# google/bayesnf

Measured on AMD Instinct MI355X. Metric: train-steps/sec x ensemble_size (member-steps/s, whole job), higher is better.
Workload: dtype bf16; 1 GPU; C2 chickenpox-like MAP: N=10232 rows, D=3, F=57, width=512, depth=2, NORMAL, full batch, lr=0.005; members_per_gpu=64, ensemble_size=64, parallelism=ensemble-shard x1 (no data-path collective)

## Files before the change

bayesnf_amd/_native.py:

```python

from __future__ import annotations

import ctypes as C
import os

import numpy as np

from . import spec as _spec

_LIB_NAME = 'libbnf_hip.so'
_lib = None

ABI_VERSION = 6
MAX_INPUTS, MAX_GROUPS, MAX_LAYERS, MAX_FREQS, MAX_INTERACT = 8, 12, 8, 96, 16
DTYPE = {'fp32': 0, 'f32': 0, 'float32': 0, 'fp32_exact': 0, 'fp32_split': 3, 'bf16x3': 3, 'bf16': 1, 'bfloat16': 1, 'fp8': 2}
DTYPE_NAME = {0: 'fp32', 1: 'bf16', 2: 'fp8', 3: 'fp32_split'}
OBS = {'NORMAL': 0, 'NB': 1, 'ZINB': 2}
MODE_MAP, MODE_VI = 0, 1
PIPELINE = {'auto': 0, 'layers': 1, 'panel': 3}

EXPORTS = (
    'bnf_abi_version', 'bnf_last_error', 'bnf_create', 'bnf_destroy',
    'bnf_workspace_bytes', 'bnf_state_bytes', 'bnf_param_bytes', 'bnf_owned_bytes', 'bnf_bind',
    'bnf_init_params', 'bnf_init_params_keys', 'bnf_train', 'bnf_row_tables', 'bnf_row_keys', 'bnf_vi_posterior_draws', 'bnf_vi_noise_keys', 'bnf_forward',
    'bnf_normal_mixture_quantiles', 'bnf_count_mixture_quantiles', 'bnf_debug_loss_and_grad',
    'bnf_debug_row_index', 'bnf_debug_vi_eps', 'bnf_debug_vi_noise', 'bnf_debug_activation',
    'bnf_debug_gemm_nt', 'bnf_debug_gemm_tn', 'bnf_debug_poison_lds', 'bnf_profile_enable', 'bnf_profile_read',
    'bnf_kernel_flops', 'bnf_comm_available', 'bnf_comm_unique_id', 'bnf_comm_create', 'bnf_allgather',
    'bnf_comm_create_local', 'bnf_allgather_group', 'bnf_comm_destroy')


class BnfConfig(C.Structure):
  _fields_ = [
      ('abi_version', C.c_int32), ('device', C.c_int32), ('dtype', C.c_int32),
      ('obs_model', C.c_int32), ('mode', C.c_int32),
      ('n_inputs', C.c_int32), ('width', C.c_int32), ('depth', C.c_int32),
      ('n_features', C.c_int32), ('n_params', C.c_int32),
      ('n_groups', C.c_int32),
      ('group_kind', C.c_int32 * MAX_GROUPS),
      ('group_arg', C.c_int32 * MAX_GROUPS),
      ('group_ncols', C.c_int32 * MAX_GROUPS),
      ('group_col0', C.c_int32 * MAX_GROUPS),
      ('group_scale_off', C.c_int32 * MAX_GROUPS),
      ('fourier_degree', C.c_int32 * MAX_INPUTS),
      ('input_scale', C.c_float * MAX_INPUTS),
      ('n_freqs', C.c_int32),
      ('freq', C.c_float * MAX_FREQS),
      ('harmonic', C.c_float * MAX_FREQS),
      ('n_interact', C.c_int32),
      ('interact', (C.c_int32 * 2) * MAX_INTERACT),
      ('off_log_noise_scale', C.c_int32), ('off_shape', C.c_int32),
      ('off_inflated', C.c_int32),
      ('off_bias', C.c_int32 * (MAX_LAYERS + 1)),
      ('off_kernel', C.c_int32 * (MAX_LAYERS + 1)),
      ('off_layer_scale', C.c_int32 * MAX_LAYERS),
      ('off_output_scale', C.c_int32), ('off_lsa', C.c_int32),
      ('off_act_weight', C.c_int32),
      ('n_rows', C.c_int64), ('batch', C.c_int64),
      ('members', C.c_int32), ('member_offset', C.c_int64),
      ('vi_samples', C.c_int32), ('forward_only', C.c_int32), ('pipeline', C.c_int32),
      ('learning_rate', C.c_float), ('prior_weight', C.c_float),
      ('kl_weight', C.c_float),
      ('seed', C.c_uint64),
  ]


def library_path() -> str:
  override = os.environ.get('BNF_LIB')
  if override:
    return override
  return os.path.join(os.path.dirname(os.path.abspath(__file__)), _LIB_NAME)


def load():
  global _lib
  if _lib is not None:
    return _lib
  path = library_path()
  if not os.path.exists(path):
    raise RuntimeError(
        f'{path} not found. Build it with `python -c "import __graft_entry__ '
        'as g; g.build()"` or `make -C bayesnf_amd/csrc`. bayesnf_amd has no '
        'CPU fallback.')
  lib = C.CDLL(path)
  vp, i32, i64, f32p = C.c_void_p, C.c_int32, C.c_int64, C.c_void_p
  lib.bnf_abi_version.restype = C.c_int
  lib.bnf_last_error.restype = C.c_char_p
  lib.bnf_create.argtypes = [C.POINTER(BnfConfig), C.POINTER(vp)]
  lib.bnf_destroy.argtypes = [vp]
  lib.bnf_destroy.restype = None
  for name in ('bnf_workspace_bytes', 'bnf_state_bytes', 'bnf_param_bytes', 'bnf_owned_bytes'):
    getattr(lib, name).argtypes = [vp]
    getattr(lib, name).restype = C.c_size_t
  lib.bnf_bind.argtypes = [vp, vp, vp, vp, vp, vp, vp]
  lib.bnf_init_params.argtypes = [vp, C.c_float]
  lib.bnf_train.argtypes = [vp, i64, i64, f32p]
  lib.bnf_comm_unique_id.argtypes = [vp]
  lib.bnf_comm_create.argtypes = [vp, i32, i32, i32, C.POINTER(vp)]
  lib.bnf_allgather.argtypes = [vp, vp, vp, C.c_size_t, vp]
  lib.bnf_comm_available.argtypes = []
  lib.bnf_comm_create_local.argtypes = [i32, C.POINTER(C.c_int32), C.POINTER(vp)]
  lib.bnf_allgather_group.argtypes = [i32, C.POINTER(vp), C.POINTER(vp), C.POINTER(vp), C.c_size_t, C.POINTER(vp)]
  lib.bnf_comm_destroy.argtypes = [vp]
  lib.bnf_comm_destroy.restype = None
  lib.bnf_vi_posterior_draws.argtypes = [vp, i32, f32p]
  lib.bnf_forward.argtypes = [vp, vp, i64, vp, i64, vp, vp]
  lib.bnf_normal_mixture_quantiles.argtypes = [
      vp, vp, vp, i64, i64, C.POINTER(C.c_float), i32, i32, vp]
  lib.bnf_count_mixture_quantiles.argtypes = [
      vp, vp, vp, i64, i64, C.POINTER(C.c_float), i32, vp, vp]
  lib.bnf_debug_loss_and_grad.argtypes = [vp, i64, i64, vp, vp]
  lib.bnf_debug_row_index.argtypes = [vp, i64, i64, vp]
  lib.bnf_debug_vi_eps.argtypes = [vp, i64, vp]
  lib.bnf_debug_vi_noise.argtypes = [vp, vp]
  lib.bnf_debug_poison_lds.argtypes = [vp, C.c_uint32]
  lib.bnf_row_tables.argtypes = [vp, vp, i64, i64]
  lib.bnf_row_keys.argtypes = [vp, vp, i64, i64, C.c_int32]
  lib.bnf_init_params_keys.argtypes = [vp, vp, C.POINTER(C.c_int32), C.c_int32, C.c_float]
  lib.bnf_vi_noise_keys.argtypes = [vp, vp, i64, vp, i64, vp, C.c_int32]
  lib.bnf_debug_activation.argtypes = [vp, i32, vp]
  lib.bnf_debug_gemm_nt.argtypes = [vp, vp, vp, i32, i32, i32, vp]
  lib.bnf_debug_gemm_tn.argtypes = [vp, vp, vp, i32, i32, i32, vp]
  lib.bnf_profile_enable.argtypes = [vp, C.c_char_p]
  lib.bnf_profile_read.argtypes = [
      vp, C.POINTER(i32), C.POINTER(C.c_char_p), C.POINTER(C.c_double),
      C.POINTER(i64)]
  lib.bnf_kernel_flops.argtypes = [vp, C.c_char_p]
  lib.bnf_kernel_flops.restype = C.c_double
  for name in EXPORTS:
    getattr(lib, name)
  if lib.bnf_abi_version() != ABI_VERSION:
    raise RuntimeError('libbnf_hip.so ABI version mismatch')
  _lib = lib
  return lib


def last_error() -> str:
  return load().bnf_last_error().decode('utf-8', 'replace')


def check(rc: int, what: str):
  if rc == 0:
    return
  msg = f'{what}: {last_error()} (code {rc})'
  if rc == -1:
    raise ValueError(msg)
  raise RuntimeError(msg)


_comm_cache = {}
_local_comm_cache = {}


def _agree(ok: bool, world: int, device, on_dev: bool) -> bool:
  import torch
  if world <= 1:
    return ok
  flag = torch.tensor([1 if ok else 0], dtype=torch.int32)
  flag = flag.to(device) if on_dev else flag
  torch.distributed.all_reduce(flag, op=torch.distributed.ReduceOp.MIN)
  return int(flag.item()) == 1


def allgather(send, recv, world: int, rank: int, lib=None):
  import torch
  lib = load() if lib is None else lib
  dev = send.device.index if send.is_cuda else -1
  key = (world, rank, dev, id(lib))
  if _comm_cache.get(key) is None:
    on_dev = send.is_cuda and world > 1 and torch.distributed.get_backend() == 'nccl'
    buf = (C.c_char * 128)()
    rc = lib.bnf_comm_available() if hasattr(lib, 'bnf_comm_available') else 0
    if rc == 0 and rank == 0:
      rc = lib.bnf_comm_unique_id(buf)
    err = None if rc == 0 else (last_error() if hasattr(lib, 'bnf_last_error') else f'code {rc}')
    if not _agree(rc == 0, world, send.device, on_dev):
      raise RuntimeError('RCCL is not reachable through libbnf_hip.so on at least one rank' + (f' (here: {err})' if err else ''))
    ident = torch.frombuffer(bytearray(buf.raw), dtype=torch.uint8).clone()
    if world > 1:
      carrier = ident.to(send.device) if on_dev else ident
      torch.distributed.broadcast(carrier, src=0)
      ident = carrier.cpu()
    comm = C.c_void_p()
    raw = (C.c_char * 128).from_buffer_copy(bytes(ident.numpy().tobytes()))
    rc = lib.bnf_comm_create(raw, world, rank, max(dev, 0), C.byref(comm))
    err = None if rc == 0 else (last_error() if hasattr(lib, 'bnf_last_error') else f'code {rc}')
    if rc == 0:
      _comm_cache[key] = comm
    if not _agree(rc == 0, world, send.device, on_dev):
      if rc == 0:
        lib.bnf_comm_destroy(_comm_cache.pop(key))
      raise RuntimeError('bnf_comm_create failed on at least one rank' + (f' (here: {err})' if err else ''))
  stream = torch.cuda.current_stream(send.device).cuda_stream if send.is_cuda else 0
  check(lib.bnf_allgather(_comm_cache[key], C.c_void_p(send.data_ptr()), C.c_void_p(recv.data_ptr()),
                          C.c_size_t(send.numel() * send.element_size()), C.c_void_p(stream)), 'bnf_allgather')


def allgather_local(sends, recvs, lib=None):
  import torch
  lib = load() if lib is None else lib
  n = len(sends)
  devs = tuple((t.device.index if t.is_cuda else i) for i, t in enumerate(sends))
  key = (devs, id(lib))
# ... 101 lines not shown
```

bayesnf_amd/csrc/bnf_api.hip:

```cpp
#include <hip/hip_runtime.h>
#include <cstring>
#include <rocprim/device/device_radix_sort.hpp>
#include <rocprim/device/device_segmented_radix_sort.hpp>

#include <dlfcn.h>

#include <atomic>
#include <cmath>
#include <cstdarg>
#include <cstdio>
#include <cstdlib>
#include <cstring>
#include <string>
#include <vector>

#include "../../include/bnf.h"
#include "bnf_gemm.h"
#include "bnf_kernels.h"
#include "bnf_panel.h"
#include "bnf_gemm8.h"

using namespace bnf;

static thread_local char g_err[512] = "";
static int fail(int code, const char* fmt, ...) {
  va_list ap;
  va_start(ap, fmt);
  vsnprintf(g_err, sizeof(g_err), fmt, ap);
  va_end(ap);
  return code;
}
#define HIPCHK(expr)                                                                   \
  do {                                                                                 \
    hipError_t _e = (expr);                                                            \
    if (_e != hipSuccess)                                                              \
      return fail(BNF_ERR_HIP, "%s failed: %s (%s:%d)", #expr, hipGetErrorString(_e), \
                  __FILE__, __LINE__);                                                 \
  } while (0)

enum KernelId {
  KID_PACK = 0, KID_FEAT, KID_FWD0, KID_FWD, KID_ROWLOSS, KID_LASTBWD, KID_DGRAD, KID_DGRAD0,
  KID_FEATBWD, KID_WGRAD0, KID_WGRAD, KID_ADAM, KID_VISAMPLE, KID_VIADAM, KID_FWDLAST, KID_PANEL, KID_COUNT
};
static const char* kKernelNames[KID_COUNT] = {
    "pack_weights", "featurize", "gemm_fwd_l0", "gemm_fwd", "row_loss", "last_bwd", "gemm_dgrad",
    "gemm_dgrad0", "feat_bwd", "gemm_wgrad_l0", "gemm_wgrad", "adam_map", "vi_sample", "vi_adam",
    "gemm_fwd_last", "panel_fwd_bwd"};

struct TimedLaunch {
  int kid;
  hipEvent_t t0, t1;
};

static constexpr int64_t kAtPad = 128;

struct bnf_handle {
  bnf_config cfg;
  NetDev nd;
  FreqTab ft;
  bool bf16 = false;
  int f32_split = 0;
  bool q8 = false;
  bool c8 = false;
  uint8_t* Wf8[BNF_MAX_LAYERS] = {}; uint8_t* Wb8[BNF_MAX_LAYERS] = {};
  uint8_t* H0q = nullptr;
  float* qscale = nullptr;
  int es = 4;
  int Ev = 0;
  int S = 1;
  int L = 0, W = 0, F = 0, Fp = 0, P = 0;
  int Wt = 0;
  bool pad = false;
  int64_t Pf = 0, Pp = 0;
  float* gradf = nullptr;
  float* theta_pad = nullptr;
  int32_t* pad_src = nullptr;
  int32_t* fold_src = nullptr;
  std::vector<int32_t> pad_src_h, fold_src_h;
  int32_t* fbmeta = nullptr;
  std::vector<int32_t> fbmeta_h;
  int fb_in_group = -1;
  int64_t N = 0, B = 0, Bp = 0;
  hipStream_t stream = nullptr;
  hipStream_t stream2 = nullptr;
  hipEvent_t ev_dz[BNF_MAX_LAYERS] = {};
  hipEvent_t ev_wg = nullptr;
  bool overlap = false;
  bool bound = false;
  int64_t adam_t = 0;
  float* params = nullptr;
  float* state = nullptr;
  char* ws = nullptr;
  const float* X = nullptr;
  const float* y = nullptr;
  float* theta_c = nullptr;
  float* grad = nullptr;
  float* stab = nullptr;
  float* stab_pred = nullptr;
  void* H0 = nullptr; void* H0t = nullptr;
  const float* ext_eps = nullptr;
  const uint32_t* vi_keys = nullptr; int64_t vi_key_rows = 0, vi_key_t0 = 0;
  const uint32_t* vi_draw_keys = nullptr; int64_t vi_draw_rows = 0;
  const int32_t* row_tab = nullptr; int64_t row_tab_epochs = 0, row_tab_e0 = 0;
  const uint32_t* row_keys = nullptr; int64_t row_keys_epochs = 0, row_keys_e0 = 0; int32_t row_key_rounds = 0;
  uint32_t* perm_bits[2] = {nullptr, nullptr}; int32_t* perm_val[2] = {nullptr, nullptr};
  unsigned* perm_seg = nullptr; void* perm_tmp = nullptr; size_t perm_tmp_bytes = 0;
  bool perm_ready = false;
  size_t owned_bytes = 0;
  int32_t* perm = nullptr; int64_t perm_epoch = -1;
  int32_t* leaf_off = nullptr; uint8_t* leaf_id = nullptr; int32_t n_leaves = 0;
  bool adam_clear_all = false;
  bool h0l = false;
  bool fold0 = false;
  void* A[BNF_MAX_LAYERS]; void* H[BNF_MAX_LAYERS]; void* Ht[BNF_MAX_LAYERS];
  void* dZ[BNF_MAX_LAYERS]; void* dZt[BNF_MAX_LAYERS];
  void* Kn[BNF_MAX_LAYERS]; void* Kt[BNF_MAX_LAYERS];
  int64_t pack_batch[BNF_MAX_LAYERS];
  float* dH0 = nullptr; float* out = nullptr; float* ybat = nullptr; float* loss_raw = nullptr;
  float* vacc = nullptr; float* dv = nullptr;
  bool vi_sample_pack = true, vi_keep_z = false;
  bool panel = false;
  void* Wf[BNF_MAX_LAYERS]; void* Wb[BNF_MAX_LAYERS];
  void* park[BNF_MAX_LAYERS];
    unsigned long long* prof_buf = nullptr;
  double prof_gap[16] = {0, 0, 0, 0, 0, 0, 0, 0, 0, 0, 0, 0, 0, 0, 0, 0};
  double prof_blocks = 0;
  int prof_threads = 0;
  bool recompute_a0 = false;
  bool fuse_last = false;
  int num_cus = 256;
  int tn_ring = 1;
  int skinny = 1;
  int big_tiles = 1;
  float* scal = nullptr;
  StepState* step_state = nullptr;
  hipGraphExec_t graph_exec = nullptr;
  int64_t graph_cols = 0;
  float* graph_losses = nullptr;
  int graph_mode = 0;
  float* qscratch = nullptr;
  float* dbg_a = nullptr; float* dbg_b = nullptr;
  uint8_t* is_matrix = nullptr;
  size_t ws_bytes = 0;
  int ablate = 0;
  uint32_t prof = 0;
  std::vector<TimedLaunch> timed;
  std::vector<hipEvent_t> event_pool;
  size_t pool_used = 0;
  double acc_ms[KID_COUNT];
  int64_t acc_calls[KID_COUNT];
};

static inline int64_t align_up(int64_t v, int64_t a) { return (v + a - 1) / a * a; }

static bool panel_h0l(const bnf_handle* h) {
  const bool shape = ((h->W == 512 || h->W == 1024) && h->Fp == 64) || (h->W == 256 && (h->Fp == 64 || h->Fp == 128));
  return h->panel && shape && !getenv("BNF_PANEL_NO_H0L");
}

static size_t carve(bnf_handle* h, char* base) {
  size_t off = 0;
  auto take = [&](size_t bytes) -> char* {
    char* p = base ? base + off : nullptr;
    off += (size_t)align_up((int64_t)bytes, 256);
    return p;
  };
  const int64_t Ev = h->Ev, Bp = h->Bp, W = h->W, Fp = h->Fp, P = h->P, es = h->es;
  const int nf2 = 2 * h->ft.n;
  const bool fo = h->cfg.forward_only != 0;
  h->grad = fo ? nullptr : (float*)take((size_t)Ev * P * 4);
  h->gradf = h->grad;
  if (h->pad) {
    h->theta_pad = (float*)take((size_t)Ev * h->Pp * 4);
    if (!fo) h->gradf = (float*)take((size_t)Ev * h->Pp * 4);
    h->pad_src = (int32_t*)take((size_t)(h->Pp - P) * 4);
    h->fold_src = (int32_t*)take((size_t)P * 4);
  }
  if (h->cfg.mode == BNF_MODE_VI) h->theta_c = (float*)take((size_t)Ev * P * 4);
  h->stab = (float*)take((size_t)std::max<int64_t>(1, h->N * nf2) * 4);
  h->stab_pred = (float*)take((size_t)std::max<int64_t>(1, Bp * nf2) * 4);
  h->H0 = take((size_t)Ev * Bp * Fp * es);
  h->H0q = (h->q8 && !fo) ? (uint8_t*)take((size_t)Ev * Bp * Fp) : nullptr;
  h->qscale = (h->q8 && !fo) ? (float*)take((size_t)Ev * 4) : nullptr;
  h->h0l = panel_h0l(h);
  h->H0t = (h->panel && !h->h0l) ? take((size_t)Ev * Bp * Fp * es) : nullptr;
  for (int l = 0; l < h->L; ++l) {
    h->A[l] = (h->panel || (h->fuse_last && l == h->L - 1) || (h->recompute_a0 && l == 0)) ? nullptr : take((size_t)Ev * W * (Bp + kAtPad) * es);
    h->H[l] = (l < h->L - 1) ? take((size_t)Ev * Bp * W * es) : nullptr;
    h->Ht[l] = nullptr;
    h->dZ[l] = fo ? nullptr : take((size_t)Ev * Bp * W * es);
    h->dZt[l] = nullptr;
    const int64_t npad = (l == 0) ? Fp : W;
    h->pack_batch[l] = npad * W;
    h->Kn[l] = h->panel ? nullptr : take((size_t)Ev * npad * W * es);
    h->Kt[l] = h->panel ? nullptr : take((size_t)Ev * npad * W * es);
  }
  for (int l = 0; l < h->L; ++l) {
    const int64_t npad = (l == 0) ? Fp : W;
    h->Wf[l] = h->panel ? take((size_t)Ev * npad * W * es) : nullptr;
    h->Wb[l] = h->panel ? take((size_t)Ev * npad * W * es) : nullptr;
    h->park[l] = (h->panel && !fo && l >= 1 && l < h->L - 1) ? take((size_t)Ev * Bp * W * es) : nullptr;
    h->Wf8[l] = (h->c8 && l >= 1) ? (uint8_t*)take((size_t)Ev * W * W) : nullptr;
    h->Wb8[l] = (h->c8 && l >= 1) ? (uint8_t*)take((size_t)Ev * W * W) : nullptr;
// ... 139 lines not shown

template <typename T, int EPI, int TAG>
static void launch_gemm(bnf_handle* h, int kid, GemmArgs g, const EpiArgs& ep) {
  if constexpr (sizeof(T) == 2 && EPI == EPI_FWD) {
    if (g.N % 256 == 0 && g.M >= 256 && h->big_tiles && (g.K >= 256 || h->big_tiles == 2)) {
      launch_gemm_wg<T, EPI, TAG, 4, 4>(h, kid, g, ep);
      return;
    }
  }
  launch_gemm_wg<T, EPI, TAG, 2, 2>(h, kid, g, ep);
}

template <typename T>
static bool fused_last_supported(int W) {
  return W == 64 || W == 128 || W == 256 || (W == 512 && sizeof(T) == 2);
}
template <typename T, int TAG>
static void launch_fwd_last_obs(bnf_handle* h, GemmArgs g, const EpiArgs& ep) {
  switch (g.N) {
    case 64: launch_gemm_wg<T, EPI_LAST, TAG, 2, 1>(h, KID_FWDLAST, g, ep); break;
    case 128: launch_gemm_wg<T, EPI_LAST, TAG, 2, 2>(h, KID_FWDLAST, g, ep); break;
    case 256: launch_gemm_wg<T, EPI_LAST, TAG, 2, 4>(h, KID_FWDLAST, g, ep); break;
    case 512:
      if constexpr (sizeof(T) == 2) launch_gemm_wg<T, EPI_LAST, TAG, 1, 8>(h, KID_FWDLAST, g, ep);
      break;
  }
}
template <typename T>
static void launch_fwd_last(bnf_handle* h, GemmArgs g, const EpiArgs& ep) {
  if (ep.obs == BNF_OBS_NORMAL) launch_fwd_last_obs<T, 3>(h, g, ep);
  else launch_fwd_last_obs<T, 4>(h, g, ep);
}

template <typename T, int TAG, int WG>
static void launch_gemm_tn_wg(bnf_handle* h, int kid, GemmArgs g, const EpiArgs& ep, hipStream_t st) {
  constexpr int kLds = gemm_tn_lds<T>(WG);
  g.tiles_m = (g.M + 64 * WG - 1) / (64 * WG);
  g.tiles_n = (g.N + 64 * WG - 1) / (64 * WG);
  if (g.splitk < 1) g.splitk = 1;
  if constexpr (std::is_same<T, float>::value) {
    if (h->f32_split) {
      static std::atomic<uint64_t> attr_done_s{0};
      allow_lds(h, &gemm_tn<T, TAG, WG, true>, kLds, &attr_done_s);
      const unsigned blocks = (unsigned)(g.members * g.tiles_m * g.tiles_n * g.splitk);
      LaunchScope ls(h, kid, st, true);
      hipLaunchKernelGGL((gemm_tn<T, TAG, WG, true>), dim3(blocks), dim3(64 * WG * WG), kLds, st, g, ep);
      return;
    }
  }
  static std::atomic<uint64_t> attr_done{0};
  allow_lds(h, &gemm_tn<T, TAG, WG>, kLds, &attr_done);
  const unsigned blocks = (unsigned)(g.members * g.tiles_m * g.tiles_n * g.splitk);
  LaunchScope ls(h, kid, st, true);
  hipLaunchKernelGGL((gemm_tn<T, TAG, WG>), dim3(blocks), dim3(64 * WG * WG), kLds, st, g, ep);
}
enum { WG_TN128 = 0, WG_TN256 = 1, WG_RING = 2, WG_SKINNY = 3 };
static void launch_gemm_tn_skinny(bnf_handle* h, int kid, GemmArgs g, const EpiArgs& ep, hipStream_t st) {
  g.tiles_m = 1;
  g.tiles_n = g.N / 512;
  if (g.splitk < 1) g.splitk = 1;
  static std::atomic<uint64_t> attr_done{0};
  allow_lds(h, &gemm_tn_skinny, kSkLds, &attr_done);
  const unsigned blocks = (unsigned)((int64_t)g.members * g.tiles_n * g.splitk);
  LaunchScope ls(h, kid, st, true);
  hipLaunchKernelGGL(gemm_tn_skinny, dim3(blocks), dim3(512), kSkLds, st, g, ep);
}
template <typename T, int TAG>
static void launch_gemm_tn(bnf_handle* h, int kid, GemmArgs g, const EpiArgs& ep, hipStream_t st, int kind) {
  if constexpr (sizeof(T) == 2 && TAG == 0) {
    if (kind == WG_SKINNY) {
      launch_gemm_tn_skinny(h, kid, g, ep, st);
      return;
    }
  }
  if constexpr (sizeof(T) == 2) {
    if (kind == WG_RING) {
      g.tiles_m = g.M / 256; g.tiles_n = g.N / 256;
      if (g.splitk < 1) g.splitk = 1;
      static std::atomic<uint64_t> attr_done{0}, attr_done_s{0};
      const unsigned blocks = (unsigned)(g.members * g.tiles_m * g.tiles_n * g.splitk * (g.n_multi > 1 ? g.n_multi : 1));
      EpiArgs ep2 = ep;
      ep2.ablate = h->ablate;
      LaunchScope ls(h, kid, st, true);
      if (g.splitk == 1) {
        allow_lds(h, &gemm_tn_ring<TAG, true>, kRgLds, &attr_done_s);
        hipLaunchKernelGGL((gemm_tn_ring<TAG, true>), dim3(blocks), dim3(512), kRgLds, st, g, ep2);
      } else {
        allow_lds(h, &gemm_tn_ring<TAG, false>, kRgLds, &attr_done);
        hipLaunchKernelGGL((gemm_tn_ring<TAG, false>), dim3(blocks), dim3(512), kRgLds, st, g, ep2);
      }
      return;
    }
  }
  if (kind == WG_TN256) {
    launch_gemm_tn_wg<T, TAG, 4>(h, kid, g, ep, st);
    return;
  }
  launch_gemm_tn_wg<T, TAG, 2>(h, kid, g, ep, st);
}

template <int TAG>
static void launch_gemm_tn8(bnf_handle* h, int kid, GemmArgs g, const EpiArgs& ep, hipStream_t st, int kind) {
  if (g.splitk < 1) g.splitk = 1;
  EpiArgs ep2 = ep;
  ep2.ablate = h->ablate;
  LaunchScope ls(h, kid, st, true);
  if (kind == WG_SKINNY && TAG == 0) {
    g.tiles_m = 1; g.tiles_n = g.N / 512;
    static std::atomic<uint64_t> attr_done{0};
    allow_lds(h, &gemm_tn_skinny8, kSk8Lds, &attr_done);
    hipLaunchKernelGGL(gemm_tn_skinny8, dim3((unsigned)((int64_t)g.members * g.tiles_n * g.splitk)), dim3(512), kSk8Lds, st, g, ep2);
  } else if (kind == WG_RING) {
    g.tiles_m = g.M / 256; g.tiles_n = g.N / 256;
    static std::atomic<uint64_t> attr_done{0}, attr_done_s{0};
    const unsigned blocks = (unsigned)(g.members * g.tiles_m * g.tiles_n * g.splitk * (g.n_multi > 1 ? g.n_multi : 1));
    if (g.splitk == 1) {
      allow_lds(h, &gemm_tn_ring8<TAG, true>, kRgLds, &attr_done_s);
      hipLaunchKernelGGL((gemm_tn_ring8<TAG, true>), dim3(blocks), dim3(512), kRgLds, st, g, ep2);
    } else {
      allow_lds(h, &gemm_tn_ring8<TAG, false>, kRgLds, &attr_done);
      hipLaunchKernelGGL((gemm_tn_ring8<TAG, false>), dim3(blocks), dim3(512), kRgLds, st, g, ep2);
    }
  } else {
    g.tiles_m = (g.M + 127) / 128; g.tiles_n = (g.N + 127) / 128;
    static std::atomic<uint64_t> attr_done{0};
    allow_lds(h, &gemm_tn8<TAG>, kTn8Lds, &attr_done);
    hipLaunchKernelGGL((gemm_tn8<TAG>), dim3((unsigned)(g.members * g.tiles_m * g.tiles_n * g.splitk)), dim3(256), kTn8Lds, st, g, ep2);
  }
}

static inline unsigned cdiv(int64_t a, int64_t b) { return (unsigned)((a + b - 1) / b); }

template <typename T>
static void run_pack(bnf_handle* h, const float* theta, int nmem) {
  LaunchScope ls(h, KID_PACK);
  PackWJobs jb{};
  jb.n_layers = h->L;
  int tiles = 0;
  for (int l = 0; l < h->L; ++l) {
    jb.off_kernel[l] = h->nd.off_kernel[l];
    jb.n_in[l] = (l == 0) ? h->F : h->W;
    jb.n_pad[l] = (l == 0) ? h->Fp : h->W;
    jb.tile0[l] = tiles;
    tiles += (jb.n_pad[l] / 32) * (h->W / 32);
    jb.Kn[l] = h->Kn[l]; jb.Kt[l] = h->Kt[l]; jb.pack_batch[l] = h->pack_batch[l];
  }
  jb.tile0[h->L] = tiles;
  hipLaunchKernelGGL((k_pack_weights<T>), dim3((unsigned)tiles, (unsigned)nmem), dim3(256), 0, h->stream, theta,
                     (int64_t)h->Pf, jb, (int32_t)h->W, (int32_t)(sizeof(T) == 4 && h->f32_split ? 1 : 0), h->nd, h->scal);
}

template <typename T>
static void run_forward(bnf_handle* h, const float* theta, int nmem, const RowSrc& rs,
                        const float* X, const float* stab, const float* y, int64_t rows,
                        bool train) {
  const int64_t Bp = h->Bp;
  {
    LaunchScope ls(h, KID_FEAT);
    dim3 grid(cdiv(rows, kFeatRows) * (unsigned)nmem);
    const size_t lds = (size_t)kFeatRows * (h->Fp + 16 / h->es) * h->es;
    static std::atomic<uint64_t> attr_done{0};
    allow_lds(h, &k_featurize<T>, 160 * 1024, &attr_done);
    hipLaunchKernelGGL((k_featurize<T>), grid, dim3(kFeatRows), lds, h->stream, h->nd, rs, X, stab,
                       y, h->scal, rows, (T*)h->H0, Bp * h->Fp,
                       (T*)nullptr, (int64_t)h->Fp * Bp, (int32_t)Bp,
                       train ? h->ybat : (float*)nullptr, Bp, (int32_t)nmem, (int32_t)0);
  }
  const int n_layers = (train && h->fuse_last) ? h->L - 1 : h->L;
  for (int l = 0; l < n_layers; ++l) {
    const bool last = l == h->L - 1;
    GemmArgs g{};
    g.A = (l == 0) ? h->H0 : h->H[l - 1];
// ... 198 lines not shown
    ep.loss = sink.loss; ep.loss_raw = sink.raw; ep.loss_stride = sink.stride; ep.S = h->S;
    ep.loss_scale = sink.scale; ep.lik_c = c; ep.st = sink.st;
    ep.off_os = h->nd.off_os; ep.off_bias_out = h->nd.off_bias[L];
    ep.off_lns = h->nd.off_lns; ep.off_shape = h->nd.off_shape; ep.off_infl = h->nd.off_infl;
    ep.obs = h->nd.obs;
    launch_fwd_last<T>(h, g, ep);
    wgrad_after_dz<T>(h, nmem, L - 1);
  } else {
    {
      RowLossArgs a{};
      a.theta = theta; a.theta_stride = h->Pf; a.B = rows;
      a.vacc = h->vacc; a.vacc_batch = Bp; a.ybat = h->ybat;
      a.out = h->out; a.out_batch = Bp; a.dv = h->dv;
      a.grad = h->gradf; a.grad_stride = h->Pf;
      a.loss = sink.loss; a.loss_stride = sink.stride; a.S = h->S; a.loss_scale = sink.scale;
      a.c = c; a.loss_raw = sink.raw; a.st = sink.st;
      LaunchScope ls(h, KID_ROWLOSS);
      hipLaunchKernelGGL((k_row_loss<true>), dim3(cdiv(rows, 256), (unsigned)nmem), dim3(256), 0,
                         h->stream, h->nd, a);
    }
    {
      LastBwdArgs a{};
      a.theta = theta; a.theta_stride = h->Pf;
      a.At = h->A[L - 1]; a.dZ = h->dZ[L - 1];
      a.act_batch = Bp * h->W; a.actt_batch = (int64_t)h->W * (Bp + kAtPad); a.ldt = (int32_t)(Bp + kAtPad);
      a.dv = h->dv; a.dv_batch = Bp; a.grad = h->gradf; a.grad_stride = h->Pf;
      a.n_row_tiles = (int32_t)((rows + 63) / 64);
      a.tiles_per_task = 4;
      const int tasks = (h->W / 64) * ((a.n_row_tiles + a.tiles_per_task - 1) / a.tiles_per_task);
      {
        LaunchScope ls(h, KID_LASTBWD);
        hipLaunchKernelGGL((k_last_bwd<T>), dim3(cdiv(tasks, 4), (unsigned)nmem), dim3(256), 0, h->stream,
                           h->nd, a);
      }
      wgrad_after_dz<T>(h, nmem, L - 1);
    }
}
  for (int l = L - 1; l >= 0; --l) {
    GemmArgs g{};
    g.A = h->dZ[l]; g.a_ld = h->W; g.a_batch = Bp * h->W;
    g.B = h->Kn[l]; g.b_ld = h->W; g.b_batch = h->pack_batch[l];
    g.M = (int)rows; g.K = h->W; g.splitk = 1; g.members = nmem;
    EpiArgs ep{};
    ep.theta = theta; ep.theta_stride = h->Pf;
    ep.grad = h->gradf; ep.grad_stride = h->Pf;
    if (l > 0) {
      g.N = h->W;
      ep.scale = 1.0f / sqrtf((float)h->Wt);
      ep.off_bias = h->nd.off_bias[l - 1];
      ep.off_layer_scale = h->nd.off_ls[l - 1];
      ep.off_act_weight = h->nd.off_law;
      ep.scal = h->scal; ep.scal_stride = kScalStride; ep.layer = l - 1;
      ep.in_a = h->A[l - 1];
      ep.out_h = h->dZ[l - 1];
      ep.act_batch = Bp * h->W; ep.actt_batch = (int64_t)h->W * (Bp + kAtPad);
      ep.ld = h->W; ep.ldt = (int32_t)(Bp + kAtPad);
      if (l == 1 && h->recompute_a0) {
        ep.aux_a = h->H0; ep.aux_a_batch = Bp * h->Fp;
        ep.aux_b = h->Kt[0]; ep.aux_b_batch = h->pack_batch[0];
        ep.aux_ld = h->Fp; ep.aux_scale = 1.0f / sqrtf((float)h->F);
        launch_gemm<T, EPI_DGRAD, 2>(h, KID_DGRAD, g, ep);
      } else {
        launch_gemm<T, EPI_DGRAD, 1>(h, KID_DGRAD, g, ep);
      }
      wgrad_after_dz<T>(h, nmem, l - 1);
    } else {
      g.N = h->Fp;
      ep.scale = 1.0f / sqrtf((float)h->F);
      ep.out_f32 = h->dH0; ep.f32_batch = (int64_t)h->Fp * Bp; ep.ld_f32 = (int32_t)Bp;
      launch_gemm<T, EPI_DGRAD0, 0>(h, KID_DGRAD0, g, ep);
    }
  }
  {
    LaunchScope ls(h, KID_FEATBWD);
    dim3 grid(cdiv(rows, 256), (unsigned)nmem);
    const float* X = h->X;
    hipLaunchKernelGGL(k_feat_bwd, grid, dim3(256), 0, h->stream, h->nd, rs, X, h->stab, theta,
                       (int64_t)h->Pf, h->scal, rows, h->dH0, (int64_t)h->Fp * Bp, (int32_t)Bp, h->gradf,
                       (int64_t)h->Pf);
  }
  wgrad_join(h);
}

static PackJobs pack_jobs(const bnf_handle* h, int* n_tiles) {
  PackJobs jb{};
  jb.n_layers = h->L; jb.W = h->W;
  int tiles = 0;
  for (int l = 0; l < h->L; ++l) {
    jb.off_kernel[l] = h->nd.off_kernel[l];
    jb.n_in[l] = (l == 0) ? h->F : h->W;
    jb.n_pad[l] = (l == 0) ? h->Fp : h->W;
    jb.tile0[l] = tiles;
    tiles += (jb.n_pad[l] / 64) * (h->W / 64);
    jb.wf[l] = h->Wf[l]; jb.wb[l] = h->Wb[l]; jb.batch[l] = h->pack_batch[l];
  }
  jb.tile0[h->L] = tiles;
  jb.fold0 = h->fold0 ? 1 : 0; jb.F0n = h->F; jb.off_bias0 = h->nd.off_bias[0]; jb.off_ls0 = h->nd.off_ls[0];
  for (int l = 0; l < h->L; ++l) { jb.wf8[l] = h->Wf8[l]; jb.wb8[l] = h->Wb8[l]; }
  jb.batch8 = (int64_t)h->W * h->W;
  *n_tiles = tiles;
  return jb;
}
template <typename T>
static void run_pack_fragments(bnf_handle* h, const float* theta, int nmem) {
  LaunchScope ls(h, KID_PACK);
  int tiles = 0;
  const PackJobs jb = pack_jobs(h, &tiles);
  hipLaunchKernelGGL((k_pack_layers<T>), dim3((unsigned)tiles * (unsigned)nmem), dim3(256), 0, h->stream,
                     theta, (int64_t)h->Pf, jb, h->nd, h->scal);
}

template <int WN, int RT, bool H0L, bool DEEP, int CH, int FP, bool F0, bool C8 = false>
static void launch_panel_f(bnf_handle* h, const PanelArgs& pa) {
  constexpr int kLds = panel_lds_bytes(WN, RT, H0L, CH, FP);
  static_assert(kLds <= 160 * 1024, "LDS per workgroup");
  static std::atomic<uint64_t> attr_done{0};
  allow_lds(h, &k_panel_fwd_bwd<WN, RT, H0L, DEEP, CH, FP, F0, C8>, kLds, &attr_done);
  PanelArgs pa2 = pa;
  pa2.ablate = h->ablate;
  const unsigned blocks = (unsigned)(pa.members * pa.panels);
  {
    EpiArgs tmp{};
    phase_prof_begin(h, KID_PANEL, blocks, &tmp);
    pa2.prof = tmp.prof;
  }
  {
    LaunchScope ls(h, KID_PANEL);
    hipLaunchKernelGGL((k_panel_fwd_bwd<WN, RT, H0L, DEEP, CH, FP, F0, C8>), dim3(blocks), dim3(512), kLds, h->stream, pa2);
  }
  phase_prof_end(h, KID_PANEL, blocks, 512);
}
template <int WN, int RT, bool H0L, bool DEEP, int CH, int FP>
static void launch_panel_d(bnf_handle* h, const PanelArgs& pa) {
  if constexpr (H0L) {
    if (h->fold0) {
      if (pa.c8) {
        launch_panel_f<WN, RT, H0L, DEEP, CH, FP, true, true>(h, pa);
        return;
      }
      launch_panel_f<WN, RT, H0L, DEEP, CH, FP, true>(h, pa);
      return;
    }
  }
  launch_panel_f<WN, RT, H0L, DEEP, CH, FP, false>(h, pa);
}

template <int WN, int RT, bool H0L, int CH = 1, int FP = 64>
static void launch_panel(bnf_handle* h, const PanelArgs& pa) {
  if (pa.n_layers == 2) launch_panel_d<WN, RT, H0L, false, CH, FP>(h, pa);
  else launch_panel_d<WN, RT, H0L, true, CH, FP>(h, pa);
}

static void run_panel(bnf_handle* h, const float* theta, int nmem, const RowSrc& rs, float c,
                      const LossSink& sink, bool fragments_packed = false) {
  const int64_t Bp = h->Bp;
  if (!fragments_packed) run_pack_fragments<bf16_t>(h, theta, nmem);
  {
    LaunchScope ls(h, KID_FEAT);
    dim3 grid(cdiv(h->B, kFeatRows) * (unsigned)nmem);
    const size_t lds = (size_t)kFeatRows * (h->Fp + 8) * 2;
    static std::atomic<uint64_t> attr_done{0};
    allow_lds(h, &k_featurize<bf16_t>, 160 * 1024, &attr_done);
    hipLaunchKernelGGL((k_featurize<bf16_t>), grid, dim3(kFeatRows), lds, h->stream, h->nd, rs, h->X, h->stab,
                       h->y, h->scal, h->B, (bf16_t*)h->H0, Bp * h->Fp, (bf16_t*)h->H0t,
                       (int64_t)h->Fp * Bp, (int32_t)Bp, h->ybat, Bp, (int32_t)nmem, (int32_t)(h->fold0 ? 2 : 0), h->H0q);
  }
  bool feat_bwd_fused = false;
  PanelArgs pa{};
  pa.F = h->F; pa.Fp = h->Fp; pa.B = (int32_t)h->B; pa.members = nmem; pa.Wt = h->Wt;
  pa.theta = theta; pa.theta_stride = h->Pf; pa.scal = h->scal;
  const int L = h->L;
  pa.n_layers = L;
  for (int l = 0; l < L; ++l) {
    pa.off_bias[l] = h->nd.off_bias[l]; pa.off_ls[l] = h->nd.off_ls[l];
    pa.Wf[l] = (const bf16_t*)h->Wf[l]; pa.Wb[l] = (const bf16_t*)h->Wb[l];
    pa.Hout[l] = (bf16_t*)h->H[l]; pa.dZ[l] = (bf16_t*)h->dZ[l]; pa.park[l] = (bf16_t*)h->park[l];
  }
  pa.off_bias_out = h->nd.off_bias[L]; pa.off_ko = h->nd.off_kernel[L];
  pa.off_os = h->nd.off_os; pa.off_law = h->nd.off_law; pa.off_lns = h->nd.off_lns;
  pa.off_shape = h->nd.off_shape; pa.off_infl = h->nd.off_infl; pa.obs = h->nd.obs;
  pa.H0 = (const bf16_t*)h->H0t; pa.H0rm = (const bf16_t*)h->H0; pa.h0_batch = Bp * h->Fp;
  pa.w0_batch = h->pack_batch[0]; pa.w1_batch = h->pack_batch[1];
  pa.act_batch = Bp * h->W;
  pa.dH0t = h->dH0; pa.dh0_batch = (int64_t)h->Fp * Bp; pa.ldt = (int32_t)Bp;
  pa.ybat = h->ybat; pa.row_batch = Bp; pa.out = h->out; pa.out_batch = Bp;
  pa.grad = h->gradf; pa.grad_stride = h->Pf;
  pa.loss = sink.loss; pa.loss_raw = sink.raw; pa.loss_stride = sink.stride; pa.S = h->S;
  pa.loss_scale = sink.scale; pa.lik_c = c; pa.st = sink.st;
  pa.q8 = h->q8 ? 1 : 0; pa.qscale = h->qscale;
  pa.c8 = h->c8 ? 1 : 0; pa.w8_batch = (int64_t)h->W * h->W;
  for (int l = 0; l < L; ++l) { pa.Wf8[l] = h->Wf8[l]; pa.Wb8[l] = h->Wb8[l]; }
  auto with_fused_featbwd = [&]() {
    pa.fbmeta = h->fbmeta; pa.off_lsa = h->nd.off_lsa; pa.n_groups = h->nd.n_groups; pa.n_inputs = h->nd.D;
    pa.fb_in_group = h->fb_in_group;
    feat_bwd_fused = h->fbmeta != nullptr;
  };
  if (h->W == 1024) {
    pa.panels = (int32_t)(Bp / panel_rows(8, 2));
    if (h->h0l) {
      with_fused_featbwd();
      launch_panel<8, 2, true, 2>(h, pa);
    } else {
      launch_panel<8, 2, false, 2>(h, pa);
    }
  } else if (h->W == 512) {
    pa.panels = (int32_t)(Bp / panel_rows(8, 4));
    if (h->h0l) {
      with_fused_featbwd();
      launch_panel<8, 4, true>(h, pa);
    } else {
      launch_panel<8, 4, false>(h, pa);
    }
  } else if (h->h0l) {
    pa.panels = (int32_t)(Bp / panel_rows(4, 2));
    with_fused_featbwd();
    if (h->Fp == 128) launch_panel<4, 2, true, 1, 128>(h, pa);
    else launch_panel<4, 2, true, 1, 64>(h, pa);
  } else {
    pa.panels = (int32_t)(Bp / panel_rows(4, 4));
    launch_panel<4, 4, false>(h, pa);
  }
  if (!feat_bwd_fused)
  {
    LaunchScope ls(h, KID_FEATBWD);
    dim3 grid(cdiv(h->B, 256), (unsigned)nmem);
    hipLaunchKernelGGL(k_feat_bwd, grid, dim3(256), 0, h->stream, h->nd, rs, h->X, h->stab, theta,
                       (int64_t)h->Pf, h->scal, h->B, h->dH0, (int64_t)h->Fp * Bp, (int32_t)Bp, h->gradf,
                       (int64_t)h->Pf);
  }
  run_wgrad<bf16_t>(h, nmem);
}

static const float* fw_theta(bnf_handle* h, const float* theta, int nmem) {
  if (!h->pad) return theta;
  hipLaunchKernelGGL(k_pad_params, dim3(cdiv(h->Pp, 256), (unsigned)nmem), dim3(256), 0, h->stream, theta,
                     (int64_t)h->P, h->theta_pad, h->Pp, h->pad_src);
  return h->theta_pad;
}
static void fold_grad(bnf_handle* h, int nmem) {
// ... 36 lines not shown
  return rs;
}

static size_t row_perm_bytes(int64_t members, int64_t n_rows) {
  return 4 * (size_t)members * (size_t)n_rows * 4 + (size_t)(members + 1) * sizeof(unsigned);
}
static int perm_members(const bnf_handle* h) { return h->cfg.mode == BNF_MODE_VI ? 1 : h->cfg.members; }
static int ensure_row_perm(bnf_handle* h, int64_t epoch) {
  if (!h->row_keys || h->B >= h->N || epoch < h->row_keys_e0 || epoch >= h->row_keys_e0 + h->row_keys_epochs) return BNF_OK;
  if (h->row_tab && epoch >= h->row_tab_e0 && epoch < h->row_tab_e0 + h->row_tab_epochs) return BNF_OK;
  if (h->perm_epoch == epoch) return BNF_OK;
  const int E = perm_members(h), R = h->row_key_rounds;
  const int64_t N = h->N, total = (int64_t)E * N;
  const bool segmented = N <= (1 << 17);
  if (!h->perm_ready) {
    uint32_t* bits[2] = {nullptr, nullptr}; int32_t* val[2] = {nullptr, nullptr};
    unsigned* seg = nullptr; void* tmp = nullptr; size_t tmp_bytes = 0;
    auto release = [&]() {
      for (int k = 0; k < 2; ++k) { if (bits[k]) (void)hipFree(bits[k]); if (val[k]) (void)hipFree(val[k]); }
      if (seg) (void)hipFree(seg);
      if (tmp) (void)hipFree(tmp);
    };
    hipError_t ae = hipSuccess;
    for (int k = 0; k < 2 && ae == hipSuccess; ++k) {
      ae = hipMalloc((void**)&bits[k], (size_t)total * 4);
      if (ae == hipSuccess) ae = hipMalloc((void**)&val[k], (size_t)total * 4);
    }
    if (ae == hipSuccess) ae = hipMalloc((void**)&seg, (size_t)(E + 1) * sizeof(unsigned));
    if (ae == hipSuccess) {
      std::vector<unsigned> off((size_t)E + 1);
      for (int e = 0; e <= E; ++e) off[(size_t)e] = (unsigned)((int64_t)e * N);
      ae = hipMemcpy(seg, off.data(), off.size() * sizeof(unsigned), hipMemcpyHostToDevice);
    }
    if (ae == hipSuccess) {
      size_t bytes = 0;
      if (segmented)
        ae = rocprim::segmented_radix_sort_pairs(nullptr, bytes, bits[0], bits[1], val[0], val[1], (unsigned)total,
                                                 (unsigned)E, seg, seg + 1, 0, 32, h->stream);
      else
        ae = rocprim::radix_sort_pairs(nullptr, bytes, bits[0], bits[1], val[0], val[1], (size_t)N, 0, 32, h->stream);
      tmp_bytes = std::max<size_t>(bytes, 16);
    }
    if (ae == hipSuccess) ae = hipMalloc(&tmp, tmp_bytes);
    if (ae != hipSuccess) {
      release();
      (void)hipGetLastError();
      return fail(BNF_ERR_HIP, "bnf_row_keys: work buffers for %d members x %lld rows (%.1f MB): %s", E, (long long)N,
                  (double)row_perm_bytes(E, N) / 1e6, hipGetErrorString(ae));
    }
    for (int k = 0; k < 2; ++k) { h->perm_bits[k] = bits[k]; h->perm_val[k] = val[k]; }
    h->perm_seg = seg; h->perm_tmp = tmp; h->perm_tmp_bytes = tmp_bytes;
    h->owned_bytes += 4 * (size_t)total * 4 + (size_t)(E + 1) * sizeof(unsigned) + tmp_bytes;
    h->perm_ready = true;
  }
  const uint32_t* keys = h->row_keys + ((epoch - h->row_keys_e0) * E) * (int64_t)R * 2;
  int cur = 0;
  for (int r = 0; r < R; ++r) {
    const unsigned half = (unsigned)((N + 1) / 2);
    hipLaunchKernelGGL(k_jax_perm_bits, dim3(cdiv(half, 256), (unsigned)E), dim3(256), 0, h->stream, keys, R, r,
                       (uint32_t)N, h->perm_bits[0], r == 0 ? h->perm_val[cur] : (int32_t*)nullptr);
    hipError_t se = hipSuccess;
    if (segmented) {
      size_t bytes = h->perm_tmp_bytes;
      se = rocprim::segmented_radix_sort_pairs(h->perm_tmp, bytes, h->perm_bits[0], h->perm_bits[1], h->perm_val[cur],
                                               h->perm_val[cur ^ 1], (unsigned)total, (unsigned)E, h->perm_seg,
                                               h->perm_seg + 1, 0, 32, h->stream);
    } else {
      for (int e = 0; e < E && se == hipSuccess; ++e) {
        size_t bytes = h->perm_tmp_bytes;
        se = rocprim::radix_sort_pairs(h->perm_tmp, bytes, h->perm_bits[0] + (int64_t)e * N, h->perm_bits[1] + (int64_t)e * N,
                                       h->perm_val[cur] + (int64_t)e * N, h->perm_val[cur ^ 1] + (int64_t)e * N, (size_t)N,
                                       0, 32, h->stream);
      }
    }
    if (se != hipSuccess) return fail(BNF_ERR_HIP, "radix sort: %s", hipGetErrorString(se));
    cur ^= 1;
  }
  h->perm = h->perm_val[cur];
  h->perm_epoch = epoch;
  HIPCHK(hipGetLastError());
  return BNF_OK;
}

template <typename T>
static int step_map(bnf_handle* h, int64_t epoch, int64_t step, const LossSink& sink, bool apply) {
  if (const int prc = ensure_row_perm(h, epoch)) return prc;
  const RowSrc rs = make_rowsrc(h, epoch, step);
  const int E = h->cfg.members;
  const float c = (float)((double)h->N / (double)h->B);
  const float* thf = fw_theta(h, h->params, E);
  if (h->panel) {
    run_panel(h, thf, E, rs, c, sink);
  } else {
    run_pack<T>(h, thf, E);
    run_forward<T>(h, thf, E, rs, h->X, h->stab, h->y, h->B, true);
    run_backward<T>(h, thf, E, rs, h->B, c, sink);
  }
  fold_grad(h, E);
  AdamArgs a{};
  a.theta = h->params; a.m = h->state; a.v = h->state + (int64_t)E * h->P; a.grad = h->grad;
  a.stride = h->P; a.P = h->P; a.off_shape = h->nd.off_shape;
  const int64_t t = h->adam_t + 1;
  a.lr = h->cfg.learning_rate;
  a.bc1 = (float)(1.0 - std::pow(0.9, (double)t));
  a.bc2 = (float)(1.0 - std::pow(0.999, (double)t));
  a.prior_weight = h->cfg.prior_weight;
  a.loss = sink.loss; a.loss_stride = sink.stride; a.loss_scale = sink.scale;
  a.apply = apply ? 1 : 0; a.loss_raw = sink.raw; a.st = sink.st;
  a.keep_lo = a.keep_hi = 0;
  if (!h->pad && !h->adam_clear_all && h->ablate == 0)
    for (int l = 1; l < h->L; ++l)
      if (wgrad_splitk(h, E, l) == 1 && a.keep_hi == 0) {
        a.keep_lo = (h->nd.off_kernel[l] + 3) / 4 * 4;
        a.keep_hi = (h->nd.off_kernel[l] + h->W * h->W) / 4 * 4;
      }
  {
    LaunchScope ls(h, KID_ADAM);
    hipLaunchKernelGGL(k_adam_map, dim3(cdiv(cdiv(h->P, 4), 256 * BNF_ADAM_QUADS), (unsigned)E), dim3(256), 0, h->stream, a);
  }
  if (apply) h->adam_t = t;
  return BNF_OK;
}

static ViSegs vi_segments_all(const bnf_handle* h) {
  ViSegs sg{};
  sg.n = 1; sg.lo[0] = 0; sg.hi[0] = h->P;
  return sg;
}
static ViSegs vi_segments_between_kernels(const bnf_handle* h) {
  ViSegs sg{};
  int32_t at = 0;
  for (int l = 0; l < h->L; ++l) {
    sg.lo[sg.n] = at; sg.hi[sg.n] = h->nd.off_kernel[l]; ++sg.n;
    at = h->nd.off_kernel[l] + ((l == 0) ? h->F : h->W) * h->W;
  }
  sg.lo[sg.n] = at; sg.hi[sg.n] = h->P; ++sg.n;
  return sg;
}
static dim3 vi_sample_grid(const ViSegs& sg, int members) {
  int32_t longest = 1;
  for (int i = 0; i < sg.n; ++i) longest = std::max(longest, sg.hi[i] - sg.lo[i]);
  return dim3(cdiv(cdiv(longest, 4) + 1, 256), (unsigned)members, (unsigned)sg.n);
}
static bool vi_sample_pack_ok(const bnf_handle* h) {
  if (!h->vi_sample_pack || !h->panel || h->pad || h->W % 64 != 0) return false;
  for (int l = 0; l < h->L; ++l)
    if ((h->nd.off_kernel[l] + kEpsQuadPhase) % 4 != 0) return false;
  return true;
}

static JaxNoise jax_noise_for_step(const bnf_handle* h) {
  JaxNoise jn{};
  if (!h->vi_keys) return jn;
  jn.keys = h->vi_keys; jn.leaf_off = h->leaf_off; jn.leaf_id = h->leaf_id;
  jn.n_leaves = h->n_leaves; jn.S = h->S; jn.members = h->cfg.members;
  jn.row = h->adam_t - h->vi_key_t0;
  return jn;
}

template <typename T>
static int step_vi(bnf_handle* h, int64_t step, float* loss, int64_t loss_stride, bool apply,
                   float* gmu_out, float* grho_out) {
  if (const int prc = ensure_row_perm(h, step)) return prc;
  const RowSrc rs = make_rowsrc(h, 0, step);
  const int E = h->cfg.members, S = h->S;
  float* mu = h->params;
  float* rho = h->params + (int64_t)E * h->P;
  const JaxNoise jn = jax_noise_for_step(h);
  if (jn.keys && (jn.row < 0 || jn.row >= h->vi_key_rows))
    return fail(BNF_ERR_STATE, "VI step %lld is outside the noise-key table (%lld rows from step %lld)",
                (long long)h->adam_t, (long long)h->vi_key_rows, (long long)h->vi_key_t0);
  const bool fused = vi_sample_pack_ok(h) && !h->ext_eps && !jn.keys;
  {
    LaunchScope ls(h, KID_VISAMPLE);
    const ViSegs segs = fused ? vi_segments_between_kernels(h) : vi_segments_all(h);
    hipLaunchKernelGGL(k_vi_sample, vi_sample_grid(segs, E), dim3(256), 0, h->stream, mu, rho, h->P, S, h->cfg.seed,
                       h->cfg.member_offset, (uint64_t)step, (uint32_t)STREAM_VI_EPS, h->theta_c,
                       (int64_t)S * h->P, (int64_t)h->P, segs, h->ext_eps, jn);
    if (fused) {
      int tiles = 0;
      const PackJobs jb = pack_jobs(h, &tiles);
      ViSampleArgs sa{};
      sa.mu = mu; sa.rho = rho; sa.P = h->P; sa.S = S; sa.seed = h->cfg.seed; sa.member_offset = h->cfg.member_offset;
      sa.step = (uint64_t)step; sa.z = h->theta_c; sa.write_z = h->vi_keep_z ? 1 : 0;
      hipLaunchKernelGGL((k_vi_sample_pack<bf16_t, BNF_VI_SP_THREADS>), dim3((unsigned)tiles * (unsigned)E),
                         dim3(BNF_VI_SP_THREADS), 0, h->stream, sa, jb,
                         h->nd, h->scal);
    }
  }
  const float kl = h->cfg.kl_weight;
  const float c = (float)((double)h->N / (double)h->B / (double)kl);
  LossSink sink{loss, loss_stride, kl / (float)S, nullptr};
  const float* thf = fw_theta(h, h->theta_c, h->Ev);
  if (h->panel) {
    run_panel(h, thf, h->Ev, rs, c, sink, fused);
  } else {
    run_pack<T>(h, thf, h->Ev);
    run_forward<T>(h, thf, h->Ev, rs, h->X, h->stab, h->y, h->B, true);
    run_backward<T>(h, thf, h->Ev, rs, h->B, c, sink);
  }
  fold_grad(h, h->Ev);
// ... 90 lines not shown
    if (feat_lds > 160 * 1024) {
      const int F = h->F, es = h->es;
      delete h;
      return fail(BNF_ERR_INVALID, "%d features need %zu bytes of LDS per featurisation workgroup (limit 163840): "
                  "at most %d features with this dtype", F, feat_lds, (160 * 1024 / (kFeatRows * es) - 16 / es) / 64 * 64);
    }
  }
  NetDev& nd = h->nd;
  memset(&nd, 0, sizeof(nd));
  nd.D = cfg->n_inputs; nd.F = h->F; nd.Fp = h->Fp; nd.W = h->W; nd.Wt = h->Wt; nd.depth = h->L; nd.P = h->P;
  nd.n_groups = cfg->n_groups; nd.n_freqs = cfg->n_freqs; nd.n_interact = cfg->n_interact;
  nd.obs = cfg->obs_model;
  for (int g = 0; g < cfg->n_groups; ++g) {
    nd.group_kind[g] = cfg->group_kind[g]; nd.group_arg[g] = cfg->group_arg[g];
    nd.group_ncols[g] = cfg->group_ncols[g]; nd.group_col0[g] = cfg->group_col0[g];
    nd.group_scale_off[g] = cfg->group_scale_off[g];
    if (cfg->group_col0[g] < 0 || cfg->group_col0[g] + cfg->group_ncols[g] > h->F ||
        cfg->group_scale_off[g] < 0 || cfg->group_scale_off[g] >= h->P) {
      delete h;
      return fail(BNF_ERR_INVALID, "feature group %d out of range", g);
    }
  }
  for (int d = 0; d < cfg->n_inputs; ++d) {
    nd.fdeg[d] = cfg->fourier_degree[d];
    nd.in_scale[d] = cfg->input_scale[d];
    if (cfg->fourier_degree[d] < 0 || cfg->fourier_degree[d] > 24) {
      delete h;
      return fail(BNF_ERR_INVALID, "fourier_degree[%d]", d);
    }
  }
  for (int k = 0; k < cfg->n_interact; ++k) {
    nd.interact[k][0] = cfg->interact[k][0];
    nd.interact[k][1] = cfg->interact[k][1];
  }
  nd.off_lns = cfg->off_log_noise_scale; nd.off_shape = cfg->off_shape; nd.off_infl = cfg->off_inflated;
  for (int l = 0; l <= h->L; ++l) {
    nd.off_bias[l] = cfg->off_bias[l];
    nd.off_kernel[l] = cfg->off_kernel[l];
  }
  h->Pf = h->P;
  if (h->pad) {
    const int W = h->W, Wt = h->Wt;
    int64_t pos = h->P;
    h->fold_src_h.resize((size_t)h->P);
    for (int64_t i = 0; i < h->P; ++i) h->fold_src_h[(size_t)i] = (int32_t)i;
    auto leaf = [&](int32_t off_true, int rows_t, int cols_t, int rows_p, int cols_p) {
      const int32_t off_pad = (int32_t)pos;
      for (int r = 0; r < rows_p; ++r)
        for (int c = 0; c < cols_p; ++c) {
          const bool in = r < rows_t && c < cols_t;
          const int32_t src = in ? off_true + r * cols_t + c : -1;
          h->pad_src_h.push_back(src);
          if (in) h->fold_src_h[(size_t)src] = (int32_t)pos;
          ++pos;
        }
      return off_pad;
    };
    for (int l = 0; l < h->L; ++l) {
      nd.off_bias[l] = leaf(cfg->off_bias[l], 1, Wt, 1, W);
      const int rt = (l == 0) ? h->F : Wt, rp = (l == 0) ? h->F : W;
      nd.off_kernel[l] = leaf(cfg->off_kernel[l], rt, Wt, rp, W);
    }
    nd.off_kernel[h->L] = leaf(cfg->off_kernel[h->L], Wt, 1, W, 1);
    while (pos % 4) { h->pad_src_h.push_back(-1); ++pos; }
    h->Pp = pos; h->Pf = pos;
  }
  for (int l = 0; l < h->L; ++l) nd.off_ls[l] = cfg->off_layer_scale[l];
  nd.off_os = cfg->off_output_scale; nd.off_lsa = cfg->off_lsa; nd.off_law = cfg->off_act_weight;
  h->ft.n = cfg->n_freqs;
  for (int j = 0; j < cfg->n_freqs; ++j) {
    h->ft.f[j] = cfg->freq[j];
    h->ft.h[j] = cfg->harmonic[j];
  }
  for (int k = 0; k < KID_COUNT; ++k) { h->acc_ms[k] = 0; h->acc_calls[k] = 0; }
  if (const char* ab = getenv("BNF_ABLATE")) h->ablate = atoi(ab);
  h->num_cus = prop.multiProcessorCount > 0 ? prop.multiProcessorCount : 256;
  if (const char* bt = getenv("BNF_BIG_TILES")) h->big_tiles = atoi(bt);
  if (const char* sk = getenv("BNF_WGRAD_SKINNY")) h->skinny = atoi(sk);
  if (const char* rg = getenv("BNF_TN_RING")) h->tn_ring = atoi(rg);
  if (const char* gm = getenv("BNF_GRAPH")) h->graph_mode = atoi(gm);
  h->adam_clear_all = getenv("BNF_ADAM_CLEAR_ALL") != nullptr;
  if (const char* v = getenv("BNF_VI_SAMPLE_PACK")) h->vi_sample_pack = atoi(v) != 0;
  if (const char* v = getenv("BNF_VI_KEEP_Z")) h->vi_keep_z = atoi(v) != 0;
  {
    int want = cfg->pipeline;
    if (const char* pf = getenv("BNF_PIPELINE")) want = atoi(pf);
    if (want != 0 && want != 1 && want != 3) {
      delete h;
      return fail(BNF_ERR_INVALID, "pipeline %d (0 auto, 1 layers, 3 panel)", want);
    }
    const bool can_panel = !cfg->forward_only && h->bf16 && h->L >= 2 && (h->W == 256 || h->W == 512 || h->W == 1024) && h->Fp <= 128;
    if (want == 3 && !can_panel) {
      delete h;
      return fail(BNF_ERR_INVALID, "panel pipeline needs a bf16 training handle with depth >= 2, width 256/512/1024 and <= 128 features");
    }
    h->panel = can_panel && (want == 3 || want == 0);
    if (h->q8 && !h->panel && !cfg->forward_only) {
      delete h;
      return fail(BNF_ERR_INVALID, "dtype fp8 (fp8 operand storage for the weight gradients) needs the row-panel pipeline: "
                  "depth >= 2, width 256 / 512 / 1024 after padding to 64, <= 128 padded features");
    }
    if (h->panel) h->Bp = align_up(h->B, 256);
    h->c8 = h->q8 && h->panel && !(getenv("BNF_FP8_CONTRACT") && atoi(getenv("BNF_FP8_CONTRACT")) == 0);
    const bool fl_ok = h->bf16 ? fused_last_supported<bf16_t>(h->W) : fused_last_supported<float>(h->W);
    h->fuse_last = !cfg->forward_only && !h->panel && want == 0 && fl_ok;
    h->recompute_a0 = !cfg->forward_only && !h->panel && want == 0 && h->L >= 2 && h->Fp <= 128;
  }
  h->h0l = panel_h0l(h);
  h->fold0 = h->h0l && h->F + 2 <= h->Fp && !(getenv("BNF_PANEL_FOLD0") && atoi(getenv("BNF_PANEL_FOLD0")) == 0);
  h->c8 = h->c8 && h->fold0;
  if (h->h0l &&
      !(getenv("BNF_PANEL_FEATBWD") && atoi(getenv("BNF_PANEL_FEATBWD")) == 0)) {
    int in_group = -1;
    for (int g = 0; g < cfg->n_groups; ++g)
      if (cfg->group_kind[g] == BNF_GROUP_INPUT) in_group = g;
    if (in_group >= 0) {
      std::vector<int32_t>& m = h->fbmeta_h;
      const int Fp = h->Fp;
      m.assign(Fp * 4 + BNF_MAX_GROUPS, 0);
      auto put = [&](int col, int kind, int g, int d1, int d2, int partner, int ucol, float coef) {
        m[4 * col] = kind | (g << 8) | (d1 << 16) | (d2 << 24);
        m[4 * col + 1] = partner | (ucol << 8);
        memcpy(&m[4 * col + 2], &coef, 4);
      };
      for (int c = 0; c < Fp; ++c) put(c, kFbNone, 0xff, 0xff, 0xff, 0, 0, 0.f);
      const int cin = cfg->group_col0[in_group];
      for (int g = 0; g < cfg->n_groups; ++g) {
        const int c0 = cfg->group_col0[g], nc = cfg->group_ncols[g];
        m[4 * Fp + g] = cfg->group_scale_off[g];
        switch (cfg->group_kind[g]) {
          case BNF_GROUP_INPUT:
            for (int d = 0; d < nc; ++d) put(c0 + d, kFbInput, g, d, 0xff, 0, 0, 0.f);
            break;
          case BNF_GROUP_FOURIER: {
            const int deg = nc / 2, d = cfg->group_arg[g];
            for (int k = 0; k < deg; ++k) {
              const float w = 6.28318530717958647692f * (float)(1u << k);
              put(c0 + k, kFbFourier, g, d, 0xff, c0 + deg + k, cin + d, -w);
              put(c0 + deg + k, kFbFourier, g, d, 0xff, c0 + k, cin + d, w);
            }
            break;
          }
          case BNF_GROUP_SEASONAL:
            for (int j = 0; j < nc; ++j) put(c0 + j, kFbNone, g, 0xff, 0xff, 0, 0, 0.f);
            break;
          default:
            for (int k = 0; k < nc; ++k)
              put(c0 + k, kFbInter, g, cfg->interact[k][0], cfg->interact[k][1], 0, 0, 0.f);
        }
      }
      h->fb_in_group = in_group;
    }
  }
  h->ws_bytes = carve(h, nullptr);
  *out = h;
  return BNF_OK;
}

void bnf_destroy(bnf_handle* h) {
  if (!h) return;
  (void)hipSetDevice(h->cfg.device);
  for (auto ev : h->event_pool) hipEventDestroy(ev);
  if (h->stream2) {
    (void)hipStreamSynchronize(h->stream2);
    (void)hipStreamDestroy(h->stream2);
  }
  for (int l = 0; l < BNF_MAX_LAYERS; ++l)
    if (h->ev_dz[l]) (void)hipEventDestroy(h->ev_dz[l]);
  if (h->ev_wg) (void)hipEventDestroy(h->ev_wg);
  if (h->graph_exec) (void)hipGraphExecDestroy(h->graph_exec);
  if (h->prof_buf) {
    if (h->prof_blocks > 0) {
      fprintf(stderr, "[phase clocks] %s: %d threads/workgroup, mean cycles per workgroup: total %.0f |",
              getenv("BNF_PHASE_PROF"), h->prof_threads, h->prof_gap[0] / h->prof_blocks);
      for (int k = 1; k < 16; ++k) fprintf(stderr, " m%d %.0f", k, h->prof_gap[k] / h->prof_blocks);
      fprintf(stderr, "\n");
    }
    (void)hipFree(h->prof_buf);
  }
  for (int k = 0; k < 2; ++k) {
    if (h->perm_bits[k]) (void)hipFree(h->perm_bits[k]);
    if (h->perm_val[k]) (void)hipFree(h->perm_val[k]);
  }
  if (h->perm_seg) (void)hipFree(h->perm_seg);
  if (h->perm_tmp) (void)hipFree(h->perm_tmp);
  delete h;
}

size_t bnf_workspace_bytes(const bnf_handle* h) { return h ? h->ws_bytes : 0; }
size_t bnf_owned_bytes(const bnf_handle* h) { return h ? h->owned_bytes : 0; }
size_t bnf_param_bytes(const bnf_handle* h) {
  if (!h) return 0;
  return (size_t)h->cfg.members * h->P * 4 * (h->cfg.mode == BNF_MODE_VI ? 2 : 1);
}
size_t bnf_state_bytes(const bnf_handle* h) {
  if (!h) return 0;
  return (size_t)h->cfg.members * h->P * 4 * (h->cfg.mode == BNF_MODE_VI ? 4 : 2);
}

int bnf_bind(bnf_handle* h, void* params, void* opt_state, void* workspace, const float* X,
             const float* y, void* stream) {
  if (!h || !workspace) return fail(BNF_ERR_INVALID, "null argument");
  if (!h->cfg.forward_only && (!params || !opt_state || !X))
    return fail(BNF_ERR_INVALID, "params / opt_state / X are required for a training handle");
  HIPCHK(hipSetDevice(h->cfg.device));
  h->stream = (hipStream_t)stream;
  h->params = (float*)params;
  h->state = (float*)opt_state;
  h->ws = (char*)workspace;
  h->X = X;
  h->y = y;
  carve(h, h->ws);
  if (h->cfg.mode != BNF_MODE_VI) h->theta_c = h->params;
  HIPCHK(hipMemsetAsync(h->ws, 0, h->ws_bytes, h->stream));
  if (h->state) HIPCHK(hipMemsetAsync(h->state, 0, bnf_state_bytes(h), h->stream));
  std::vector<uint8_t> mm((size_t)h->P, 0);
  for (int l = 0; l <= h->L; ++l) {
    const int64_t n_in = (l == 0) ? h->F : h->Wt, n_out = (l == h->L) ? 1 : h->Wt;
    for (int64_t i = 0; i < n_in * n_out; ++i) mm[(size_t)h->cfg.off_kernel[l] + i] = 1;
  }
  HIPCHK(hipMemcpyAsync(h->is_matrix, mm.data(), (size_t)h->P, hipMemcpyHostToDevice, h->stream));
  if (h->fbmeta)
    HIPCHK(hipMemcpyAsync(h->fbmeta, h->fbmeta_h.data(), h->fbmeta_h.size() * 4, hipMemcpyHostToDevice, h->stream));
  if (h->pad) {
    HIPCHK(hipMemcpyAsync(h->pad_src, h->pad_src_h.data(), h->pad_src_h.size() * 4, hipMemcpyHostToDevice, h->stream));
    HIPCHK(hipMemcpyAsync(h->fold_src, h->fold_src_h.data(), h->fold_src_h.size() * 4, hipMemcpyHostToDevice, h->stream));
    if (h->gradf != h->grad) HIPCHK(hipMemsetAsync(h->gradf, 0, (size_t)h->Ev * h->Pp * 4, h->stream));
  }
  HIPCHK(hipStreamSynchronize(h->stream));
  if (h->ft.n > 0 && X) {
    hipLaunchKernelGGL(k_seasonal_table, dim3(cdiv(h->N, 256)), dim3(256), 0, h->stream, X, h->N,
                       h->nd.D, h->ft, h->stab);
  }
  HIPCHK(hipGetLastError());
  if (!h->stream2 && !h->cfg.forward_only) {
    if (const char* ov = getenv("BNF_OVERLAP")) h->overlap = atoi(ov) != 0;
    HIPCHK(hipStreamCreateWithFlags(&h->stream2, hipStreamNonBlocking));
    for (int l = 0; l < h->L; ++l) HIPCHK(hipEventCreateWithFlags(&h->ev_dz[l], hipEventDisableTiming));
    HIPCHK(hipEventCreateWithFlags(&h->ev_wg, hipEventDisableTiming));
  }
  h->bound = true;
  h->adam_t = 0;
  h->vi_keys = h->vi_draw_keys = nullptr; h->vi_key_rows = h->vi_draw_rows = 0; h->vi_key_t0 = 0;
  h->row_tab = nullptr; h->row_tab_epochs = 0;
  h->row_keys = nullptr; h->row_keys_epochs = 0; h->perm_epoch = -1;
  return BNF_OK;
}

int bnf_init_params(bnf_handle* h, float log_noise_init) {
  if (!h || !h->bound) return fail(BNF_ERR_STATE, "bnf_init_params before bnf_bind");
  if (h->cfg.forward_only || !h->params) return fail(BNF_ERR_STATE, "forward_only handle");
  HIPCHK(hipSetDevice(h->cfg.device));
  const int E = h->cfg.members;
  dim3 grid(cdiv(h->P, 256), (unsigned)E);
  hipLaunchKernelGGL(k_init_params, grid, dim3(256), 0, h->stream, h->params, h->P, h->is_matrix,
                     h->nd.off_lns, log_noise_init, h->cfg.seed, h->cfg.member_offset);
  if (h->cfg.mode == BNF_MODE_VI) {
    const int64_t n = (int64_t)E * h->P;
    hipLaunchKernelGGL(k_fill, dim3(cdiv(n, 256)), dim3(256), 0, h->stream, h->params + n, n,
                       -1.0502256128148466f);
  }
  HIPCHK(hipMemsetAsync(h->state, 0, bnf_state_bytes(h), h->stream));
  HIPCHK(hipGetLastError());
  h->adam_t = 0;
  h->vi_keys = h->vi_draw_keys = nullptr; h->vi_key_rows = h->vi_draw_rows = 0; h->vi_key_t0 = 0;
  return BNF_OK;
}

int bnf_init_params_keys(bnf_handle* h, const uint32_t* leaf_keys, const int32_t* leaf_offsets, int32_t n_leaves,
                         float log_noise_init) {
  if (!h || !h->bound) return fail(BNF_ERR_STATE, "bnf_init_params_keys before bnf_bind");
  if (h->cfg.forward_only || !h->params) return fail(BNF_ERR_STATE, "forward_only handle");
  if (!leaf_keys || !leaf_offsets || n_leaves < 1 || n_leaves > 64) return fail(BNF_ERR_INVALID, "leaf_keys / leaf_offsets / n_leaves (1..64)");
  if (leaf_offsets[0] != 0 || leaf_offsets[n_leaves] != h->P) return fail(BNF_ERR_INVALID, "leaf_offsets must cover [0, P)");
  HIPCHK(hipSetDevice(h->cfg.device));
  LeafTable lt{};
  lt.n = n_leaves;
  for (int k = 0; k <= n_leaves; ++k) lt.off[k] = leaf_offsets[k];
  const int E = h->cfg.members;
  const float ua = (float)std::erf((double)(-2.0f / 1.41421356237309504880f));
  const float ub = (float)std::erf((double)(2.0f / 1.41421356237309504880f));
  dim3 grid(cdiv(h->P, 256), (unsigned)E);
  hipLaunchKernelGGL(k_init_params_keys, grid, dim3(256), 0, h->stream, h->params, h->P, h->is_matrix, lt, leaf_keys,
                     h->nd.off_lns, log_noise_init, ua, ub);
  if (h->cfg.mode == BNF_MODE_VI) {
    const int64_t n = (int64_t)E * h->P;
    hipLaunchKernelGGL(k_fill, dim3(cdiv(n, 256)), dim3(256), 0, h->stream, h->params + n, n, -1.0502256128148466f);
  }
  HIPCHK(hipMemsetAsync(h->state, 0, bnf_state_bytes(h), h->stream));
  HIPCHK(hipGetLastError());
  h->adam_t = 0;
  h->vi_keys = h->vi_draw_keys = nullptr; h->vi_key_rows = h->vi_draw_rows = 0; h->vi_key_t0 = 0;
  return BNF_OK;
}

int bnf_train(bnf_handle* h, int64_t epoch0, int64_t num_epochs, float* losses) {
  if (!h || !h->bound) return fail(BNF_ERR_STATE, "bnf_train before bnf_bind");
  if (!losses || num_epochs < 0) return fail(BNF_ERR_INVALID, "losses / num_epochs");
  if (!h->y) return fail(BNF_ERR_STATE, "bnf_train needs a target bound");
  if (h->cfg.forward_only) return fail(BNF_ERR_STATE, "handle was created forward_only");
  HIPCHK(hipSetDevice(h->cfg.device));
  const int E = h->cfg.members;
  HIPCHK(hipMemsetAsync(losses, 0, (size_t)E * num_epochs * 4, h->stream));
  int rc = BNF_OK;
  if (h->cfg.mode == BNF_MODE_MAP) {
    const int64_t steps = h->N / h->B;
    const bool graph_ok = h->B >= h->N && !h->prof && !h->overlap && h->stream2 && num_epochs >= 8 &&
                          h->graph_mode == 1;
    if (graph_ok) {
      StepState st0{};
      st0.t = h->adam_t + 1; st0.col = 0;
      st0.bc1 = (float)(1.0 - std::pow(0.9, (double)st0.t));
      st0.bc2 = (float)(1.0 - std::pow(0.999, (double)st0.t));
      HIPCHK(hipMemcpyAsync(h->step_state, &st0, sizeof(st0), hipMemcpyHostToDevice, h->stream));
      HIPCHK(hipStreamSynchronize(h->stream));
      if (!h->graph_exec || h->graph_cols != num_epochs || h->graph_losses != losses) {
        if (h->graph_exec) { (void)hipGraphExecDestroy(h->graph_exec); h->graph_exec = nullptr; }
        hipGraph_t graph = nullptr;
        hipStream_t user_stream = h->stream;
        h->stream = h->stream2;
        const hipError_t be = hipStreamBeginCapture(h->stream, hipStreamCaptureModeRelaxed);
        if (be != hipSuccess) {
          h->stream = user_stream;
            return fail(BNF_ERR_HIP, "hipStreamBeginCapture: %s", hipGetErrorString(be));
        }
        LossSink sink{losses, num_epochs, 1.0f, nullptr, h->step_state};
        rc = h->bf16 ? step_map<bf16_t>(h, epoch0, 0, sink, true) : step_map<float>(h, epoch0, 0, sink, true);
        h->adam_t -= 1;
        hipLaunchKernelGGL(k_step_advance, dim3(1), dim3(1), 0, h->stream, h->step_state);
        const hipError_t ce = hipStreamEndCapture(h->stream, &graph);
        h->stream = user_stream;
        if (rc != BNF_OK) return rc;
        if (ce != hipSuccess) return fail(BNF_ERR_HIP, "hipStreamEndCapture: %s", hipGetErrorString(ce));
        const hipError_t ie = hipGraphInstantiate(&h->graph_exec, graph, nullptr, nullptr, 0);
        (void)hipGraphDestroy(graph);
        if (ie != hipSuccess) return fail(BNF_ERR_HIP, "hipGraphInstantiate: %s", hipGetErrorString(ie));
        h->graph_cols = num_epochs; h->graph_losses = losses;
      }
      for (int64_t ep = 0; ep < num_epochs; ++ep) HIPCHK(hipGraphLaunch(h->graph_exec, h->stream));
      h->adam_t += num_epochs;
      HIPCHK(hipGetLastError());
      return BNF_OK;
    }
    for (int64_t ep = 0; ep < num_epochs && rc == BNF_OK; ++ep) {
      for (int64_t s = 0; s < steps && rc == BNF_OK; ++s) {
        LossSink sink{losses + ep, num_epochs, 1.0f / (float)steps, nullptr};
        rc = h->bf16 ? step_map<bf16_t>(h, epoch0 + ep, s, sink, true)
                     : step_map<float>(h, epoch0 + ep, s, sink, true);
      }
    }
  } else {
    for (int64_t st = 0; st < num_epochs && rc == BNF_OK; ++st) {
      rc = h->bf16 ? step_vi<bf16_t>(h, epoch0 + st, losses + st, num_epochs, true, nullptr, nullptr)
                   : step_vi<float>(h, epoch0 + st, losses + st, num_epochs, true, nullptr, nullptr);
    }
  }
  if (rc != BNF_OK) return rc;
  HIPCHK(hipGetLastError());
  return BNF_OK;
}

int bnf_vi_posterior_draws(bnf_handle* h, int32_t n_draws, float* out) {
  if (!h || !h->bound) return fail(BNF_ERR_STATE, "not bound");
  if (h->cfg.mode != BNF_MODE_VI) return fail(BNF_ERR_STATE, "not a VI handle");
  if (n_draws < 1 || n_draws > 65535 || !out) return fail(BNF_ERR_INVALID, "n_draws/out");
  HIPCHK(hipSetDevice(h->cfg.device));
  const int E = h->cfg.members;
  JaxNoise jn{};
  if (h->vi_draw_keys) {
    if (n_draws > h->vi_draw_rows) return fail(BNF_ERR_INVALID, "n_draws exceeds the draw-key table");
    jn.keys = h->vi_draw_keys; jn.leaf_off = h->leaf_off; jn.leaf_id = h->leaf_id;
    jn.n_leaves = h->n_leaves; jn.S = n_draws; jn.members = E; jn.row = 0;
  }
  const ViSegs segs = vi_segments_all(h);
  hipLaunchKernelGGL(k_vi_sample, vi_sample_grid(segs, E), dim3(256), 0, h->stream, h->params,
                     h->params + (int64_t)E * h->P, h->P, n_draws, h->cfg.seed,
                     h->cfg.member_offset, (uint64_t)0, (uint32_t)STREAM_VI_DRAW, out, (int64_t)h->P,
                     (int64_t)E * h->P, segs, (const float*)nullptr, jn);
  HIPCHK(hipGetLastError());
  return BNF_OK;
}

int bnf_forward(bnf_handle* h, const float* theta, int64_t n_members, const float* Xnew,
                int64_t n_rows, float* loc, float* aux) {
  if (!h || !h->bound) return fail(BNF_ERR_STATE, "bnf_forward before bnf_bind");
  if (!theta || !Xnew || !loc || n_members < 1 || n_rows < 1) return fail(BNF_ERR_INVALID, "argument");
  if (h->panel) return fail(BNF_ERR_STATE, "bnf_forward needs a forward_only (or pipeline=1) handle");
  HIPCHK(hipSetDevice(h->cfg.device));
  const int64_t row_chunk = h->Bp, mem_chunk = h->Ev;
  RowSrc rs{};
  rs.mode = 0; rs.S = 1;
  for (int64_t m0 = 0; m0 < n_members; m0 += mem_chunk) {
    const int nm = (int)std::min<int64_t>(mem_chunk, n_members - m0);
    const float* th = fw_theta(h, theta + m0 * h->P, nm);
    if (h->bf16) run_pack<bf16_t>(h, th, nm); else run_pack<float>(h, th, nm);
    for (int64_t r0 = 0; r0 < n_rows; r0 += row_chunk) {
      const int64_t rows = std::min<int64_t>(row_chunk, n_rows - r0);
      const float* Xc = Xnew + r0 * h->nd.D;
      if (h->ft.n > 0)
        hipLaunchKernelGGL(k_seasonal_table, dim3(cdiv(rows, 256)), dim3(256), 0, h->stream, Xc, rows,
                           h->nd.D, h->ft, h->stab_pred);
      RowLossArgs a{};
      a.theta = th; a.theta_stride = h->Pf; a.B = rows;
      a.vacc = h->vacc; a.vacc_batch = h->Bp;
      a.out = loc + m0 * n_rows + r0; a.out_batch = n_rows;
      a.S = 1;
      if (h->bf16) run_forward<bf16_t>(h, th, nm, rs, Xc, h->stab_pred, nullptr, rows, false);
      else run_forward<float>(h, th, nm, rs, Xc, h->stab_pred, nullptr, rows, false);
      hipLaunchKernelGGL((k_row_loss<false>), dim3(cdiv(rows, 256), (unsigned)nm), dim3(256), 0,
                         h->stream, h->nd, a);
    }
  }
  if (aux)
    hipLaunchKernelGGL(k_forecast_aux, dim3(cdiv(n_members, 256)), dim3(256), 0, h->stream, theta,
                       (int64_t)h->P, (int32_t)n_members, h->nd.off_lns, h->nd.off_shape,
                       h->nd.off_infl, aux);
  HIPCHK(hipGetLastError());
  return BNF_OK;
}

int bnf_normal_mixture_quantiles(bnf_handle* h, const float* means, const float* scales,
                                 int64_t n_members, int64_t n_rows, const float* q, int32_t n_q,
                                 int32_t approximate, float* out) {
  if (!h || !h->bound) return fail(BNF_ERR_STATE, "not bound");
  if (!means || !scales || !q || !out || n_members < 1 || n_rows < 1 || n_q < 0)
    return fail(BNF_ERR_INVALID, "argument");
  HIPCHK(hipSetDevice(h->cfg.device));
  float* mpart = h->qscratch;
  float* spart = h->qscratch + 2048;
  float* bracket = h->qscratch + 4096;
  if (!approximate) {
    const int nb_m = (int)std::min<int64_t>(1024, cdiv(n_members * n_rows, 256));
    const int nb_s = (int)std::min<int64_t>(1024, cdiv(n_members, 256));
    hipLaunchKernelGGL(k_minmax_partial, dim3(nb_m), dim3(256), 0, h->stream, means,
                       n_members * n_rows, mpart);
    hipLaunchKernelGGL(k_minmax_partial, dim3(nb_s), dim3(256), 0, h->stream, scales, n_members, spart);
    hipLaunchKernelGGL(k_bracket, dim3(1), dim3(64), 0, h->stream, mpart, nb_m, spart, nb_s, bracket);
  }
  for (int i = 0; i < n_q; ++i) {
    if (approximate)
      hipLaunchKernelGGL(k_quantile_approx, dim3(cdiv(n_rows, 256)), dim3(256), 0, h->stream, means,
                         scales, n_members, n_rows, q[i], out + (int64_t)i * n_rows);
    else
      hipLaunchKernelGGL(k_quantile_root, dim3(cdiv(n_rows, 256)), dim3(256), 0, h->stream, means,
                         scales, n_members, n_rows, bracket, q[i], out + (int64_t)i * n_rows);
  }
  HIPCHK(hipGetLastError());
  return BNF_OK;
}

int bnf_count_mixture_quantiles(bnf_handle* h, const float* loc, const float* aux,
                                int64_t n_members, int64_t n_rows, const float* q, int32_t n_q,
                                float* means, float* out) {
  if (!h || !h->bound) return fail(BNF_ERR_STATE, "not bound");
  if (h->cfg.obs_model != BNF_OBS_NB && h->cfg.obs_model != BNF_OBS_ZINB)
    return fail(BNF_ERR_STATE, "handle's observation model is not NB / ZINB");
  if (!loc || !aux || !means || n_members < 1 || n_rows < 1 || n_q < 0 || (n_q > 0 && (!q || !out)))
    return fail(BNF_ERR_INVALID, "argument");
  for (int i = 0; i < n_q; ++i)
    if (!(q[i] > 0.f && q[i] < 1.f)) return fail(BNF_ERR_INVALID, "quantile %g outside (0, 1)", q[i]);
  HIPCHK(hipSetDevice(h->cfg.device));
  float* part = h->qscratch;
  float* bracket = h->qscratch + 4096;
  const int nb = (int)std::min<int64_t>(1024, cdiv(n_members * n_rows, 256));
  hipLaunchKernelGGL(k_count_moments, dim3(nb), dim3(256), 0, h->stream, loc, aux, n_members, n_rows,
                     h->cfg.obs_model, means, part);
  hipLaunchKernelGGL(k_count_bracket, dim3(1), dim3(64), 0, h->stream, part, nb, bracket);
  for (int i = 0; i < n_q; ++i)
    hipLaunchKernelGGL(k_count_quantile_root, dim3(cdiv(n_rows, 64)), dim3(64), 0, h->stream, loc, aux,
                       n_members, n_rows, h->cfg.obs_model, bracket, q[i], out + (int64_t)i * n_rows);
  HIPCHK(hipGetLastError());
  return BNF_OK;
}


int bnf_debug_loss_and_grad(bnf_handle* h, int64_t epoch, int64_t step, float* grads, float* loss) {
  if (!h || !h->bound) return fail(BNF_ERR_STATE, "not bound");
  if (h->cfg.forward_only) return fail(BNF_ERR_STATE, "forward_only handle");
  if (!grads || !loss) return fail(BNF_ERR_INVALID, "null");
  HIPCHK(hipSetDevice(h->cfg.device));
  const int E = h->cfg.members;
  int rc;
  if (h->cfg.mode == BNF_MODE_MAP) {
    HIPCHK(hipMemsetAsync(h->loss_raw, 0, (size_t)h->Ev * 4, h->stream));
    HIPCHK(hipMemsetAsync(loss, 0, (size_t)E * 4, h->stream));
    LossSink sink{loss, 1, 1.0f, nullptr};
    rc = h->bf16 ? step_map<bf16_t>(h, epoch, step, sink, false) : step_map<float>(h, epoch, step, sink, false);
    if (rc != BNF_OK) return rc;
    HIPCHK(hipMemcpyAsync(grads, h->grad, (size_t)E * h->P * 4, hipMemcpyDeviceToDevice, h->stream));
    HIPCHK(hipMemsetAsync(h->grad, 0, (size_t)h->Ev * h->P * 4, h->stream));
  } else {
    HIPCHK(hipMemsetAsync(loss, 0, (size_t)E * 4, h->stream));
    float* gmu = grads;
    float* grho = grads + (int64_t)E * h->P;
    rc = h->bf16 ? step_vi<bf16_t>(h, step, loss, 1, false, gmu, grho)
                 : step_vi<float>(h, step, loss, 1, false, gmu, grho);
    if (rc != BNF_OK) return rc;
    HIPCHK(hipMemsetAsync(h->grad, 0, (size_t)h->Ev * h->P * 4, h->stream));
  }
  HIPCHK(hipGetLastError());
  return BNF_OK;
}

int bnf_debug_row_index(bnf_handle* h, int64_t epoch, int64_t step, int32_t* out) {
  if (!h || !h->bound || !out) return fail(BNF_ERR_STATE, "not bound / null");
  HIPCHK(hipSetDevice(h->cfg.device));
  if (const int prc = ensure_row_perm(h, h->cfg.mode == BNF_MODE_VI ? step : epoch)) return prc;
  RowSrc rs = make_rowsrc(h, epoch, step);
  rs.S = 1;
  dim3 grid(cdiv(h->B, 256), (unsigned)h->cfg.members);
  hipLaunchKernelGGL(k_row_index, grid, dim3(256), 0, h->stream, rs, h->B, out);
  HIPCHK(hipGetLastError());
  return BNF_OK;
}

int bnf_vi_noise_keys(bnf_handle* h, const uint32_t* step_keys, int64_t n_steps, const uint32_t* draw_keys,
                      int64_t n_draws, const int32_t* leaf_offsets, int32_t n_leaves) {
  if (!h || !h->bound) return fail(BNF_ERR_STATE, "not bound");
  if (h->cfg.mode != BNF_MODE_VI) return fail(BNF_ERR_STATE, "not a VI handle");
  if (!step_keys && !draw_keys) {
    h->vi_keys = h->vi_draw_keys = nullptr; h->vi_key_rows = h->vi_draw_rows = 0;
    return BNF_OK;
  }
  if (!leaf_offsets || n_leaves < 1 || n_leaves > 255 || leaf_offsets[0] != 0 || leaf_offsets[n_leaves] != h->P)
    return fail(BNF_ERR_INVALID, "leaf_offsets must be n_leaves + 1 increasing offsets from 0 to P (n_leaves <= 255)");
  if ((step_keys && n_steps < 1) || (draw_keys && n_draws < 1)) return fail(BNF_ERR_INVALID, "key-table rows");
  HIPCHK(hipSetDevice(h->cfg.device));
  std::vector<uint8_t> ids((size_t)h->P);
  for (int l = 0; l < n_leaves; ++l) {
    if (leaf_offsets[l + 1] <= leaf_offsets[l]) return fail(BNF_ERR_INVALID, "leaf_offsets not increasing");
    for (int32_t p = leaf_offsets[l]; p < leaf_offsets[l + 1]; ++p) ids[(size_t)p] = (uint8_t)l;
  }
  HIPCHK(hipMemcpyAsync(h->leaf_off, leaf_offsets, (size_t)(n_leaves + 1) * 4, hipMemcpyHostToDevice, h->stream));
  HIPCHK(hipMemcpyAsync(h->leaf_id, ids.data(), (size_t)h->P, hipMemcpyHostToDevice, h->stream));
  HIPCHK(hipStreamSynchronize(h->stream));
  h->n_leaves = n_leaves;
  h->vi_keys = step_keys; h->vi_key_rows = step_keys ? n_steps : 0; h->vi_key_t0 = h->adam_t;
  h->vi_draw_keys = draw_keys; h->vi_draw_rows = draw_keys ? n_draws : 0;
  return BNF_OK;
}

int bnf_row_tables(bnf_handle* h, const int32_t* tables, int64_t epoch0, int64_t n_epochs) {
  if (!h || !h->bound) return fail(BNF_ERR_STATE, "not bound");
  if (h->cfg.mode != BNF_MODE_MAP) return fail(BNF_ERR_STATE, "row tables serve MAP / MLE epochs");
  if (!tables) { h->row_tab = nullptr; h->row_tab_epochs = 0; return BNF_OK; }
  if (n_epochs < 1 || epoch0 < 0) return fail(BNF_ERR_INVALID, "epoch0 / n_epochs");
  h->row_tab = tables; h->row_tab_e0 = epoch0; h->row_tab_epochs = n_epochs;
  return BNF_OK;
}

int bnf_row_keys(bnf_handle* h, const uint32_t* keys, int64_t epoch0, int64_t n_epochs, int32_t rounds) {
  if (!h || !h->bound) return fail(BNF_ERR_STATE, "not bound");
  h->perm_epoch = -1;
  if (!keys) { h->row_keys = nullptr; h->row_keys_epochs = 0; return BNF_OK; }
  if (n_epochs < 1 || epoch0 < 0 || rounds < 1 || rounds > 8) return fail(BNF_ERR_INVALID, "epoch0 / n_epochs / rounds");
  const int want = (int)std::ceil(3.0 * std::log((double)std::max<int64_t>(1, h->N)) / std::log(4294967295.0));
  if (rounds != want) return fail(BNF_ERR_INVALID, "rounds = %d, jax.random.permutation of %lld rows takes %d", rounds, (long long)h->N, want);
  if ((int64_t)perm_members(h) * h->N > 0x7fffffffLL)
    return fail(BNF_ERR_INVALID, "bnf_row_keys: members x rows = %lld exceeds 2^31 - 1", (long long)((int64_t)perm_members(h) * h->N));
  h->row_keys = keys; h->row_keys_e0 = epoch0; h->row_keys_epochs = n_epochs; h->row_key_rounds = rounds;
  return BNF_OK;
}

int bnf_debug_vi_noise(bnf_handle* h, const float* eps) {
  if (!h || !h->bound) return fail(BNF_ERR_STATE, "not bound");
  if (h->cfg.mode != BNF_MODE_VI) return fail(BNF_ERR_STATE, "not a VI handle");
  h->ext_eps = eps;
  return BNF_OK;
}

int bnf_debug_vi_eps(bnf_handle* h, int64_t step, float* out) {
  if (!h || !h->bound || !out) return fail(BNF_ERR_STATE, "not bound / null");
  HIPCHK(hipSetDevice(h->cfg.device));
  dim3 grid(cdiv(h->P, 256), (unsigned)h->cfg.members, (unsigned)h->S);
  JaxNoise jn = jax_noise_for_step(h);
  if (jn.keys) {
    jn.row = step - h->vi_key_t0;
    if (jn.row < 0 || jn.row >= h->vi_key_rows) return fail(BNF_ERR_INVALID, "step outside the noise-key table");
  }
  hipLaunchKernelGGL(k_vi_eps_dump, grid, dim3(256), 0, h->stream, h->P, h->cfg.seed,
                     h->cfg.member_offset, (uint64_t)step, out, jn);
  HIPCHK(hipGetLastError());
  return BNF_OK;
}

int bnf_debug_activation(bnf_handle* h, int32_t what, float* out) {
  if (!h || !h->bound || !out) return fail(BNF_ERR_STATE, "not bound / null");
  HIPCHK(hipSetDevice(h->cfg.device));
  const int64_t B = h->B, Bp = h->Bp;
  const void* src = nullptr;
  int64_t batch = 0; int ld = 0, cols = 0, transposed = 0;
  if (what == 0) { src = h->H0; batch = Bp * h->Fp; ld = h->Fp; cols = h->F; }
  else if (what >= 1 && what < h->L) { src = h->H[what - 1]; batch = Bp * h->W; ld = h->W; cols = h->Wt; }
  else if (what >= 100 && what < 100 + h->L) {
    src = h->A[what - 100]; batch = (int64_t)h->W * (Bp + kAtPad); ld = (int)(Bp + kAtPad); cols = h->Wt; transposed = 1;
  } else if (what >= 300 && what < 300 + h->L) { src = h->dZ[what - 300]; batch = Bp * h->W; ld = h->W; cols = h->Wt; }
  else if (what == 200) {
    for (int e = 0; e < h->Ev; ++e)
      HIPCHK(hipMemcpyAsync(out + (int64_t)e * B, h->out + (int64_t)e * Bp, (size_t)B * 4,
                            hipMemcpyDeviceToDevice, h->stream));
    return BNF_OK;
  } else if (what == 400) {
    dim3 grid(cdiv(B * h->F, 256), (unsigned)h->Ev);
    hipLaunchKernelGGL((k_to_f32<float>), grid, dim3(256), 0, h->stream, (const float*)h->dH0,
                       (int64_t)h->Fp * Bp, (int)Bp, B, h->F, out, 1);
    HIPCHK(hipGetLastError());
    return BNF_OK;
  } else {
    return fail(BNF_ERR_INVALID, "what=%d (the last hidden output is never stored)", what);
  }
  if (!src) return fail(BNF_ERR_STATE, "buffer not allocated on this handle");
  dim3 grid(cdiv(B * cols, 256), (unsigned)h->Ev);
  if (h->q8 && h->panel && what != 0) {
    const bool dz = what >= 300;
    hipLaunchKernelGGL(k_q8_to_f32, grid, dim3(256), 0, h->stream, (const uint8_t*)src, batch, ld, B, cols, out,
                       dz ? 1 : 0, dz ? h->qscale : (const float*)nullptr);
    HIPCHK(hipGetLastError());
    return BNF_OK;
  }
  if (h->bf16)
    hipLaunchKernelGGL((k_to_f32<bf16_t>), grid, dim3(256), 0, h->stream, (const bf16_t*)src, batch, ld, B, cols, out, transposed);
  else
    hipLaunchKernelGGL((k_to_f32<float>), grid, dim3(256), 0, h->stream, (const float*)src, batch, ld, B, cols, out, transposed);
  HIPCHK(hipGetLastError());
  return BNF_OK;
}

int bnf_debug_gemm_nt(bnf_handle* h, const float* A, const float* Bt, int32_t M, int32_t N, int32_t K,
                      float* C) {
  if (!h || !A || !Bt || !C) return fail(BNF_ERR_INVALID, "null");
  if (M < 1 || N < 1 || K < 64 || K % 64 != 0) return fail(BNF_ERR_INVALID, "K must be a multiple of 64");
  HIPCHK(hipSetDevice(h->cfg.device));
  hipStream_t st = h->stream;
  void *dA = nullptr, *dB = nullptr;
  HIPCHK(hipMalloc(&dA, (size_t)M * K * h->es));
  HIPCHK(hipMalloc(&dB, (size_t)N * K * h->es));
  GemmArgs g{};
  g.A = dA; g.B = dB; g.a_ld = K; g.b_ld = K; g.a_batch = 0; g.b_batch = 0;
  g.M = M; g.N = N; g.K = K; g.splitk = 1; g.members = 1;
  EpiArgs ep{};
  ep.scale = 1.f; ep.out_f32 = C; ep.f32_batch = 0; ep.ld_f32 = N;
  if (h->bf16) {
    hipLaunchKernelGGL((k_from_f32<bf16_t>), dim3(cdiv((int64_t)M * K, 256)), dim3(256), 0, st, A, (int64_t)M, K, (bf16_t*)dA, K);
    hipLaunchKernelGGL((k_from_f32<bf16_t>), dim3(cdiv((int64_t)N * K, 256)), dim3(256), 0, st, Bt, (int64_t)N, K, (bf16_t*)dB, K);
    launch_gemm<bf16_t, EPI_PLAIN, 2>(h, KID_FWD, g, ep);
  } else {
    hipLaunchKernelGGL((k_from_f32<float>), dim3(cdiv((int64_t)M * K, 256)), dim3(256), 0, st, A, (int64_t)M, K, (float*)dA, K);
    hipLaunchKernelGGL((k_from_f32<float>), dim3(cdiv((int64_t)N * K, 256)), dim3(256), 0, st, Bt, (int64_t)N, K, (float*)dB, K);
    launch_gemm<float, EPI_PLAIN, 2>(h, KID_FWD, g, ep);
  }
  HIPCHK(hipStreamSynchronize(st));
  HIPCHK(hipFree(dA));
  HIPCHK(hipFree(dB));
  HIPCHK(hipGetLastError());
  return BNF_OK;
}

static int debug_tn_kind(const bnf_handle* h, const GemmArgs& g) {
  if (h->big_tiles && g.M % 256 == 0 && g.N % 256 == 0 &&
      ((int64_t)g.members * (g.M / 256) * (g.N / 256) >= 128 || h->big_tiles == 2))
    return (h->bf16 && h->tn_ring && g.K % 64 == 0) ? WG_RING : WG_TN256;
  return WG_TN128;
}

int bnf_debug_gemm_tn(bnf_handle* h, const float* A, const float* B, int32_t R, int32_t M, int32_t N,
                      float* C) {
  if (!h || !A || !B || !C) return fail(BNF_ERR_INVALID, "null");
  if (R < 64 || R % 64 != 0 || M < 1 || N < 1 || M % 8 != 0 || N % 8 != 0)
    return fail(BNF_ERR_INVALID, "R must be a multiple of 64, M and N multiples of 8");
  HIPCHK(hipSetDevice(h->cfg.device));
  hipStream_t st = h->stream;
  void *dA = nullptr, *dB = nullptr;
  HIPCHK(hipMalloc(&dA, (size_t)R * M * h->es));
  HIPCHK(hipMalloc(&dB, (size_t)R * N * h->es));
  GemmArgs g{};
  g.A = dA; g.B = dB; g.a_ld = M; g.b_ld = N; g.M = M; g.N = N; g.K = R; g.splitk = 1; g.members = 1;
  EpiArgs ep{};
  ep.scale = 1.f; ep.out_f32 = C; ep.f32_batch = 0; ep.ld_f32 = N;
  if (h->q8) {
    const int kind = getenv("BNF_DEBUG_TN_KIND") ? atoi(getenv("BNF_DEBUG_TN_KIND")) : WG_TN128;
    g.splitk = getenv("BNF_DEBUG_TN_SPLITK") ? std::max(1, atoi(getenv("BNF_DEBUG_TN_SPLITK"))) : 1;
    if ((kind == WG_RING && (M % 256 || N % 256)) || (kind == WG_SKINNY && (M != 64 || N % 512)) ||
        (kind != WG_RING && kind != WG_SKINNY && kind != WG_TN128) || M % 16 || N % 16) {
      (void)hipFree(dA); (void)hipFree(dB);
      return fail(BNF_ERR_INVALID, "fp8 weight-gradient kernel kind %d does not take (M, N) = (%d, %d)", kind, M, N);
    }
    hipLaunchKernelGGL((k_from_f32_q8<false>), dim3(cdiv((int64_t)R * M, 256)), dim3(256), 0, st, A, (int64_t)R, M, (uint8_t*)dA, M);
    hipLaunchKernelGGL((k_from_f32_q8<true>), dim3(cdiv((int64_t)R * N, 256)), dim3(256), 0, st, B, (int64_t)R, N, (uint8_t*)dB, N);
    if (g.splitk > 1) HIPCHK(hipMemsetAsync(C, 0, (size_t)M * N * 4, st));
    if (kind == WG_SKINNY) launch_gemm_tn8<0>(h, KID_WGRAD0, g, ep, st, kind);
    else launch_gemm_tn8<1>(h, KID_WGRAD, g, ep, st, kind);
  } else if (h->bf16) {
    hipLaunchKernelGGL((k_from_f32<bf16_t>), dim3(cdiv((int64_t)R * M, 256)), dim3(256), 0, st, A, (int64_t)R, M, (bf16_t*)dA, M);
    hipLaunchKernelGGL((k_from_f32<bf16_t>), dim3(cdiv((int64_t)R * N, 256)), dim3(256), 0, st, B, (int64_t)R, N, (bf16_t*)dB, N);
    launch_gemm_tn<bf16_t, 2>(h, KID_WGRAD, g, ep, st, debug_tn_kind(h, g));
  } else {
    hipLaunchKernelGGL((k_from_f32<float>), dim3(cdiv((int64_t)R * M, 256)), dim3(256), 0, st, A, (int64_t)R, M, (float*)dA, M);
    hipLaunchKernelGGL((k_from_f32<float>), dim3(cdiv((int64_t)R * N, 256)), dim3(256), 0, st, B, (int64_t)R, N, (float*)dB, N);
    launch_gemm_tn<float, 2>(h, KID_WGRAD, g, ep, st, debug_tn_kind(h, g));
  }
  HIPCHK(hipStreamSynchronize(st));
  HIPCHK(hipFree(dA));
  HIPCHK(hipFree(dB));
  HIPCHK(hipGetLastError());
  return BNF_OK;
}

__global__ __launch_bounds__(1024) void k_poison_lds(uint32_t pattern, uint32_t* sink) {
  extern __shared__ uint32_t poison_sm[];
  for (int i = threadIdx.x; i < 160 * 1024 / 4; i += 1024) poison_sm[i] = pattern ^ ((uint32_t)i & 0xffu);
// ... 229 lines not shown
```

bayesnf_amd/csrc/bnf_gemm.h:

```cpp
#pragma once

#include <type_traits>

#include "bnf_device.h"

namespace bnf {

enum { EPI_FWD = 0, EPI_DGRAD = 1, EPI_DGRAD0 = 2, EPI_WGRAD = 3, EPI_PLAIN = 4, EPI_LAST = 5 };

constexpr int kBM = 128, kBN = 128, kThreads = 256;
constexpr int kGemmLds = 128 * (kBN + 4) * 4;

struct GemmArgs {
  const void* A;
  const void* B;
  int64_t a_batch, b_batch;
  int32_t a_ld, b_ld;
  int32_t M, N, K;
  int32_t tiles_m, tiles_n, splitk, members;
  int32_t n_multi;
  const void* A_multi[BNF_MAX_LAYERS]; const void* B_multi[BNF_MAX_LAYERS];
  int32_t off_out_multi[BNF_MAX_LAYERS];
};

struct EpiArgs {
  const float* theta;
  int64_t theta_stride;
  float scale;
  int32_t off_bias, off_layer_scale, off_act_weight;
  const float* scal;
  int32_t scal_stride, layer;
  void* out_a;
  void* out_h;
  const void* in_a;
  const void* aux_a;
  const void* aux_b;
  int64_t aux_a_batch, aux_b_batch;
  int32_t aux_ld;
  float aux_scale;
  float* vdot;
  int64_t vdot_batch;
  int32_t off_ko;
  float inv_sw;
  int64_t act_batch;
  int64_t actt_batch;
  int32_t ld, ldt;
  float* grad;
  int64_t grad_stride;
  int32_t off_out;
  float* out_f32;
  int64_t f32_batch;
  int32_t ld_f32;
  const float* ybat;
  float* out;
  int64_t row_batch, out_batch;
  float* loss;
  float* loss_raw;
  const StepState* st;
  int64_t loss_stride;
  int32_t S;
  float loss_scale, lik_c;
  int32_t off_os, off_bias_out, off_lns, off_shape, off_infl, obs;
  int32_t bias_row, off_bias_row;
  const float* qscale;
  unsigned long long* prof;
  int32_t ablate;
};

template <typename T>
struct Mma;

template <>
struct Mma<bf16_t> {
  static constexpr int kRowBytes = 64;
  static constexpr int kTileK = 32;
  static constexpr int kSteps = 2;
  __host__ __device__ static constexpr int stages(int wgm, int wgn) { return (wgm == 1 && wgn == 8) ? 2 : 3; }
  __host__ __device__ static constexpr int lds_bytes(int wgm, int wgn, int extra) {
    const int ring = stages(wgm, wgn) * 64 * (wgm + wgn) * kRowBytes, tile = 64 * wgm * (64 * wgn + 8) * 2 + extra;
    return ring > tile ? ring : tile;
  }
  __host__ __device__ static constexpr int min_waves(int waves) { return waves <= 4 ? 3 : 4; }
  __device__ static __forceinline__ int swz(int row) { return (row >> 2) & 3; }
  struct Frag {
    bf16x8 v;
  };
  __device__ static __forceinline__ Frag load(const char* row, int swz, int ks, int kg) {
// ... 1084 lines not shown
#pragma unroll
    for (int i = 0; i < 2; ++i) {
      const int ba = (i * 32 + pcol) * 2, bb = (wave * 64 + i * 32 + pcol) * 2;
      off_a[t][i] = lds0 + (uint32_t)(row * 128 + ((ba & ~63) ^ ((row & 1) << 6)) + (ba & 63));
      off_b[t][i] = lds0 + (uint32_t)(kSkA + row * 1024 + ((bb & ~63) ^ ((row & 3) << 6)) + (bb & 63));
    }
  }

  constexpr int kPerWave = 5;
  constexpr int kAhead = (kSkStages - 2) * kPerWave;
  constexpr int kWait = (kAhead & 15) | ((kAhead >> 4) << 14) | 0x0F70;
  constexpr int kWaitAll = 0x0F70;
#pragma unroll
  for (int s = 0; s < kSkStages - 1; ++s)
    if (kt0 + s < kt1) stage(s, kt0 + s);
  for (int ktb = kt0; ktb < kt1; ktb += kSkStages) {
#pragma unroll
    for (int sb = 0; sb < kSkStages; ++sb) {
      const int kt = ktb + sb;
      if (kt >= kt1) break;
      if (kt + kSkStages - 2 >= kt1) __builtin_amdgcn_s_waitcnt(kWaitAll);
      else __builtin_amdgcn_s_waitcnt(kWait);
      __builtin_amdgcn_s_barrier();
      if (kt + kSkStages - 1 < kt1) stage((sb + kSkStages - 1) % kSkStages, kt + kSkStages - 1);
      u32x2_t ra_[2][2][2], rb_[2][2][2];
#pragma unroll
      for (int t = 0; t < 2; ++t)
#pragma unroll
        for (int i = 0; i < 2; ++i) {
          const uint32_t aa = off_a[t][i] + sb * kSkStage, ab = off_b[t][i] + sb * kSkStage;
          ra_[0][t][i] = lds_tr16_b64<0>(aa);
          rb_[0][t][i] = lds_tr16_b64<0>(ab);
          ra_[1][t][i] = lds_tr16_b64<16 * 128>(aa);
          rb_[1][t][i] = lds_tr16_b64<16 * 1024>(ab);
        }
#pragma unroll
      for (int ks = 0; ks < kSkRows / 16; ++ks) {
        if (ks == 0) lds_tr_fence(ra_[0], rb_[0]);
        else asm volatile("" : "+v"(ra_[1][0][0]), "+v"(ra_[1][0][1]), "+v"(ra_[1][1][0]), "+v"(ra_[1][1][1]),
                               "+v"(rb_[1][0][0]), "+v"(rb_[1][0][1]), "+v"(rb_[1][1][0]), "+v"(rb_[1][1][1]));
        bf16x8 fa[2], fb[2];
#pragma unroll
        for (int i = 0; i < 2; ++i) {
          const u32x4 wa = {ra_[ks][0][i].x, ra_[ks][0][i].y, ra_[ks][1][i].x, ra_[ks][1][i].y};
          const u32x4 wb = {rb_[ks][0][i].x, rb_[ks][0][i].y, rb_[ks][1][i].x, rb_[ks][1][i].y};
          fa[i] = __builtin_bit_cast(bf16x8, wa);
          fb[i] = __builtin_bit_cast(bf16x8, wb);
        }
#pragma unroll
        for (int i = 0; i < 2; ++i)
#pragma unroll
          for (int j = 0; j < 2; ++j)
            acc[i][j] = __builtin_amdgcn_mfma_f32_32x32x16_bf16(fa[i], fb[j], acc[i][j], 0, 0, 0);
      }
    }
  }

  const int mw = 4 * kg;
  const int nw = n0 + wave * 64 + frow;
  float* out = ep.out_f32 ? ep.out_f32 + (int64_t)e * ep.f32_batch
                          : ep.grad + (int64_t)e * ep.grad_stride + ep.off_out;
#pragma unroll
  for (int j = 0; j < 2; ++j) {
    const int n = nw + j * 32;
#pragma unroll
    for (int i = 0; i < 2; ++i)
#pragma unroll
      for (int r = 0; r < 16; ++r) {
        const int m = mw + i * 32 + 8 * (r >> 2) + (r & 3);
        if (m < g.M) {
          const float v = acc[i][j][r] * ep.scale;
          if (g.splitk > 1) atomicAdd(&out[(int64_t)m * ep.ld_f32 + n], v);
          else out[(int64_t)m * ep.ld_f32 + n] = v;
        } else if (ep.bias_row && m == g.M) {
          atomicAdd(&ep.grad[(int64_t)e * ep.grad_stride + ep.off_bias_row + n], acc[i][j][r]);
        }
      }
  }
}


constexpr int kRgRows = 32, kRgStages = 4, kRgOp = kRgRows * 512, kRgStage = 2 * kRgOp;
constexpr int kRgLds = kRgStages * kRgStage;
template <int TAG, bool SWAP, int NW = 8>
__global__ __launch_bounds__(64 * NW, NW == 8 ? 2 : 1) void gemm_tn_ring(const GemmArgs g, const EpiArgs ep) {
  constexpr int TJ = NW == 8 ? 2 : 4;
  constexpr int QN = 16 / NW;
  extern __shared__ __attribute__((aligned(16))) char smem[];
  const int tid = threadIdx.x, lane = tid & 63;
  const int wave = __builtin_amdgcn_readfirstlane(tid >> 6);
  const int wr = wave / (NW / 2), wc = wave % (NW / 2);

  const int n_multi = g.n_multi > 1 ? g.n_multi : 1;
  const uint32_t per_layer = (uint32_t)(g.tiles_m * g.tiles_n * g.splitk);
  const uint32_t per_member = per_layer * (uint32_t)n_multi;
  uint32_t w = xcd_remap(blockIdx.x, gridDim.x);
  const int e = (int)(w / per_member);
  w -= (uint32_t)e * per_member;
  const int which = (int)(w / per_layer);
  w -= (uint32_t)which * per_layer;
  const int tiles = g.tiles_m * g.tiles_n;
  const int split = (int)(w / (uint32_t)tiles);
  w -= (uint32_t)split * tiles;
  const int tm = (int)(w / (uint32_t)g.tiles_n), tn = (int)(w % (uint32_t)g.tiles_n);
  const int m0 = tm * 256, n0 = tn * 256;
  const void* gA = g.A;
  const void* gB = g.B;
  int32_t off_out = ep.off_out;
#pragma unroll
  for (int k = 0; k < 8; ++k)
    if (g.n_multi > 1 && which == k) { gA = g.A_multi[k]; gB = g.B_multi[k]; off_out = g.off_out_multi[k]; }

  const int nk_total = g.K / kRgRows;
  const int nk_per = (nk_total + g.splitk - 1) / g.splitk;
  const int kt0 = split * nk_per;
  const int kt1 = min(nk_total, kt0 + nk_per);

  const char* Ab = reinterpret_cast<const char*>(gA) + (int64_t)e * g.a_batch * 2 + m0 * 2;
  const char* Bb = reinterpret_cast<const char*>(gB) + (int64_t)e * g.b_batch * 2 + n0 * 2;

  uint32_t src_a[QN], src_b[QN];
#pragma unroll
  for (int q = 0; q < QN; ++q) {
    const int srow = (wave * QN + q) * 2 + (lane >> 5);
    const uint32_t schunk = (uint32_t)(((lane & 31) ^ ((srow & 3) << 2)) * 16);
    src_a[q] = (uint32_t)srow * (uint32_t)g.a_ld * 2u + schunk;
    src_b[q] = (uint32_t)srow * (uint32_t)g.b_ld * 2u + schunk;
  }
  typedef __attribute__((address_space(3))) void lds_void_t;
  typedef __attribute__((address_space(1))) const void glb_void_t;
  auto pin = [](const char* p) {
    const uint64_t b = (uint64_t)p;
    const uint32_t lo = __builtin_amdgcn_readfirstlane((uint32_t)b);
    const uint32_t hi = __builtin_amdgcn_readfirstlane((uint32_t)(b >> 32));
    return reinterpret_cast<const char*>(((uint64_t)hi << 32) | lo);
  };
  auto stage = [&](int buf, int kt) {
    char* sA = smem + buf * kRgStage;
    char* sB = sA + kRgOp;
    const char* pa = pin(Ab + (int64_t)kt * kRgRows * g.a_ld * 2);
    const char* pb = pin(Bb + (int64_t)kt * kRgRows * g.b_ld * 2);
#pragma unroll
    for (int q = 0; q < QN; ++q) {
      dma_1k<BNF_TN_AUX>(pa, src_a[q], sA + (wave * QN + q) * 1024);
      dma_1k<BNF_TN_AUX>(pb, src_b[q], sB + (wave * QN + q) * 1024);
    }
  };

  f32x16 acc[4][TJ];
#pragma unroll
  for (int i = 0; i < 4; ++i)
#pragma unroll
    for (int j = 0; j < TJ; ++j)
#pragma unroll
      for (int r = 0; r < 16; ++r) acc[i][j][r] = 0.f;

  const int frow = lane & 31, kg = lane >> 5;
  const int p = lane & 15, half = (lane >> 4) & 1;
  const int prow = p >> 2, pcol = half * 16 + (p & 3) * 4;
  typedef __attribute__((address_space(3))) char lds_char_t;
  const uint32_t lds0 = (uint32_t)(uintptr_t)(lds_char_t*)smem;
  uint32_t off_a[4], off_b[TJ];
  {
    const int row = kg * 8 + prow;
#pragma unroll
    for (int i = 0; i < 4; ++i) {
      const int ba = (wr * 128 + i * 32 + pcol) * 2;
      off_a[i] = lds0 + (uint32_t)(row * 512 + ((ba & ~63) ^ ((row & 3) << 6)) + (ba & 63));
    }
#pragma unroll
    for (int j = 0; j < TJ; ++j) {
      const int bb = (wc * (32 * TJ) + j * 32 + pcol) * 2;
      off_b[j] = lds0 + (uint32_t)(kRgOp + row * 512 + ((bb & ~63) ^ ((row & 3) << 6)) + (bb & 63));
    }
  }
  struct Frags {
    u32x2_t a[2][4], b[2][TJ];
  };
  auto read_k = [&](Frags& f, int sb, auto ks_tag) {
    constexpr int ks = decltype(ks_tag)::value;
#pragma unroll
    for (int i = 0; i < 4; ++i) {
      f.a[0][i] = lds_tr16_b64<ks * 16 * 512>(off_a[i] + sb * kRgStage);
      f.a[1][i] = lds_tr16_b64<ks * 16 * 512 + 4 * 512>(off_a[i] + sb * kRgStage);
    }
#pragma unroll
    for (int j = 0; j < TJ; ++j) {
      f.b[0][j] = lds_tr16_b64<ks * 16 * 512>(off_b[j] + sb * kRgStage);
      f.b[1][j] = lds_tr16_b64<ks * 16 * 512 + 4 * 512>(off_b[j] + sb * kRgStage);
    }
  };
  auto fence = [&](Frags& f) {
    if constexpr (TJ == 4)
      asm volatile("" : "+v"(f.b[0][2]), "+v"(f.b[0][3]), "+v"(f.b[1][2]), "+v"(f.b[1][3]));
    asm volatile("s_waitcnt lgkmcnt(0)"
                 : "+v"(f.a[0][0]), "+v"(f.a[0][1]), "+v"(f.a[0][2]), "+v"(f.a[0][3]), "+v"(f.a[1][0]), "+v"(f.a[1][1]),
                   "+v"(f.a[1][2]), "+v"(f.a[1][3]), "+v"(f.b[0][0]), "+v"(f.b[0][1]), "+v"(f.b[1][0]), "+v"(f.b[1][1]));
    if constexpr (TJ == 4)
      asm volatile("" : "+v"(f.b[0][2]), "+v"(f.b[0][3]), "+v"(f.b[1][2]), "+v"(f.b[1][3]));
  };
  auto touch = [&](Frags& f) {
    asm volatile("" : "+v"(f.a[0][0]), "+v"(f.a[0][1]), "+v"(f.a[0][2]), "+v"(f.a[0][3]), "+v"(f.a[1][0]), "+v"(f.a[1][1]),
                      "+v"(f.a[1][2]), "+v"(f.a[1][3]), "+v"(f.b[0][0]), "+v"(f.b[0][1]), "+v"(f.b[1][0]), "+v"(f.b[1][1]));
    if constexpr (TJ == 4)
      asm volatile("" : "+v"(f.b[0][2]), "+v"(f.b[0][3]), "+v"(f.b[1][2]), "+v"(f.b[1][3]));
  };
  auto mma_k = [&](const Frags& f) {
    bf16x8 fa[4], fb[TJ];
#pragma unroll
    for (int i = 0; i < 4; ++i) {
      const u32x4 wa = {f.a[0][i].x, f.a[0][i].y, f.a[1][i].x, f.a[1][i].y};
      fa[i] = __builtin_bit_cast(bf16x8, wa);
    }
#pragma unroll
    for (int j = 0; j < TJ; ++j) {
      const u32x4 wb = {f.b[0][j].x, f.b[0][j].y, f.b[1][j].x, f.b[1][j].y};
      fb[j] = __builtin_bit_cast(bf16x8, wb);
    }
#pragma unroll
    for (int i = 0; i < 4; ++i)
#pragma unroll
      for (int j = 0; j < TJ; ++j)
        acc[i][j] = SWAP ? __builtin_amdgcn_mfma_f32_32x32x16_bf16(fb[j], fa[i], acc[i][j], 0, 0, 0)
                         : __builtin_amdgcn_mfma_f32_32x32x16_bf16(fa[i], fb[j], acc[i][j], 0, 0, 0);
    if constexpr (NW == 4) {
#pragma unroll
      for (int i = 0; i < 4; ++i)
        asm volatile("" : "+a"(acc[i][0]), "+a"(acc[i][1]), "+a"(acc[i][2]), "+a"(acc[i][3]));
    }
  };
  using K0 = std::integral_constant<int, 0>;
  using K1 = std::integral_constant<int, 1>;

  constexpr int kPerWave = 2 * QN;
  auto vm = [](int n) constexpr { return (n & 15) | ((n >> 4) << 14) | 0x0F70; };
  constexpr int kWait1 = vm(kPerWave);
  constexpr int kWaitAll = 0x0F70;
#pragma unroll
  for (int s = 0; s < kRgStages - 1; ++s)
    if (kt0 + s < kt1) stage(s, kt0 + s);
  if (kt0 + 1 < kt1) {
    if (kt0 + 2 < kt1) __builtin_amdgcn_s_waitcnt(vm(2 * kPerWave));
    else __builtin_amdgcn_s_waitcnt(kWait1);
  } else {
    __builtin_amdgcn_s_waitcnt(kWaitAll);
  }
  __builtin_amdgcn_s_barrier();
  Frags f0, f1;
  if (kt0 < kt1) {
    read_k(f0, 0, K0{});
    read_k(f1, 0, K1{});
  }
  for (int ktb = kt0; ktb < kt1; ktb += kRgStages) {
#pragma unroll(NW == 8 ? kRgStages : 1)
    for (int sb = 0; sb < kRgStages; ++sb) {
      const int kt = ktb + sb;
      if (kt >= kt1) break;
      if (kt + 2 < kt1) __builtin_amdgcn_s_waitcnt(kWait1);
      else __builtin_amdgcn_s_waitcnt(kWaitAll);
      __builtin_amdgcn_s_barrier();
      if (kt + kRgStages - 1 < kt1) stage((sb + kRgStages - 1) % kRgStages, kt + kRgStages - 1);
      fence(f0);
      touch(f1);
      const bool more = kt + 1 < kt1;
      const int sn = (sb + 1) % kRgStages;
      mma_k(f0);
      if (more) read_k(f0, sn, K0{});
      mma_k(f1);
      if (more) read_k(f1, sn, K1{});
    }
  }

  float* out = ep.out_f32 ? ep.out_f32 + (int64_t)e * ep.f32_batch
                          : ep.grad + (int64_t)e * ep.grad_stride + off_out;
  if constexpr (SWAP) {
    const int mw = m0 + wr * 128 + frow;
    const int nw = n0 + wc * (32 * TJ) + 4 * kg;
#pragma unroll
    for (int i = 0; i < 4; ++i) {
      float* orow = out + (int64_t)(mw + i * 32) * ep.ld_f32 + nw;
#pragma unroll
      for (int j = 0; j < TJ; ++j)
#pragma unroll
        for (int rg = 0; rg < 4; ++rg) {
          const float v[4] = {acc[i][j][rg * 4] * ep.scale, acc[i][j][rg * 4 + 1] * ep.scale,
                              acc[i][j][rg * 4 + 2] * ep.scale, acc[i][j][rg * 4 + 3] * ep.scale};
          store4u(orow + j * 32 + 8 * rg, 4, v);
        }
    }
  } else {
    const int mw = m0 + wr * 128 + 4 * kg;
    const int nw = n0 + wc * (32 * TJ) + frow;
#pragma unroll
    for (int j = 0; j < TJ; ++j) {
      const int n = nw + j * 32;
#pragma unroll
      for (int i = 0; i < 4; ++i)
#pragma unroll
        for (int r = 0; r < 16; ++r) {
          const int m = mw + i * 32 + 8 * (r >> 2) + (r & 3);
          const float v = acc[i][j][r] * ep.scale;
          if (g.splitk > 1) atomicAdd(&out[(int64_t)m * ep.ld_f32 + n], v);
          else out[(int64_t)m * ep.ld_f32 + n] = v;
        }
    }
  }
}


}
```

bayesnf_amd/csrc/bnf_kernels.h:

```cpp
#pragma once

#include "bnf_device.h"
#include "../../include/bnf.h"

namespace bnf {

constexpr int kScalGroup = BNF_MAX_LAYERS + 2;
constexpr int kScalInput = kScalGroup + BNF_MAX_GROUPS;
constexpr int kScalGfac = kScalInput + BNF_MAX_INPUTS;
constexpr int kScalStride = kScalGfac + BNF_MAX_GROUPS;

__device__ __forceinline__ void sincos_rev(float x, float* s, float* c) {
  sincosf(6.28318530717958647692f * x, s, c);
}

struct NetDev {
  int32_t D, F, Fp, W, Wt, depth, P, n_groups, n_freqs, n_interact, obs;
  int32_t group_kind[BNF_MAX_GROUPS], group_arg[BNF_MAX_GROUPS], group_ncols[BNF_MAX_GROUPS],
      group_col0[BNF_MAX_GROUPS], group_scale_off[BNF_MAX_GROUPS];
  int32_t fdeg[BNF_MAX_INPUTS];
  float in_scale[BNF_MAX_INPUTS];
  int32_t interact[BNF_MAX_INTERACT][2];
  int32_t off_lns, off_shape, off_infl;
  int32_t off_bias[BNF_MAX_LAYERS + 1], off_kernel[BNF_MAX_LAYERS + 1], off_ls[BNF_MAX_LAYERS];
// ... 493 lines not shown
      const uint16_t hi = f32_to_bf16_bits(v);
      q[p & 7] = hi;
      q[8 + (p & 7)] = f32_to_bf16_bits(v - bf16_bits_to_f32(hi));
      return;
    }
  }
  Elem<T>::store(row + p, v);
}

struct PackWJobs {
  int32_t n_layers;
  int32_t off_kernel[BNF_MAX_LAYERS], n_in[BNF_MAX_LAYERS], n_pad[BNF_MAX_LAYERS], tile0[BNF_MAX_LAYERS + 1];
  void* Kn[BNF_MAX_LAYERS];
  void* Kt[BNF_MAX_LAYERS];
  int64_t pack_batch[BNF_MAX_LAYERS];
};

template <typename T>
__global__ __launch_bounds__(256) void k_pack_weights(const float* __restrict__ theta, int64_t theta_stride, PackWJobs jb,
                                                      int32_t W, int32_t split, NetDev nd, float* __restrict__ scal) {
  __shared__ float tile[32][33];
  const int e = blockIdx.y;
  if (blockIdx.x == 0 && threadIdx.x == 0 && scal)
    member_scalars_row(nd, theta + (int64_t)e * theta_stride, scal + (int64_t)e * kScalStride);
  int l = 0;
  while (l + 1 < jb.n_layers && (int)blockIdx.x >= jb.tile0[l + 1]) ++l;
  const int bx = (int)blockIdx.x - jb.tile0[l];
  const int n_in = jb.n_in[l], n_pad = jb.n_pad[l];
  const int tiles_j = W / 32;
  const int ti = bx / tiles_j, tj = bx % tiles_j;
  const int tx = threadIdx.x & 31, ty = threadIdx.x >> 5;
  const float* K = theta + (int64_t)e * theta_stride + jb.off_kernel[l];
  T* kn = reinterpret_cast<T*>(jb.Kn[l]) + (int64_t)e * jb.pack_batch[l];
  T* kt = reinterpret_cast<T*>(jb.Kt[l]) + (int64_t)e * jb.pack_batch[l];
#pragma unroll
  for (int s = 0; s < 4; ++s) {
    const int i = ti * 32 + ty + s * 8, j = tj * 32 + tx;
    const float v = (i < n_in) ? K[(int64_t)i * W + j] : 0.f;
    tile[ty + s * 8][tx] = v;
    if (i < n_pad) store_packed(kn + (int64_t)i * W, j, v, split);
  }
  __syncthreads();
#pragma unroll
  for (int s = 0; s < 4; ++s) {
    const int j = tj * 32 + ty + s * 8, i = ti * 32 + tx;
    if (i < n_pad) store_packed(kt + (int64_t)j * n_pad, i, tile[tx][ty + s * 8], split);
  }
}

__global__ void k_pad_params(const float* __restrict__ theta, int64_t P, float* __restrict__ theta_pad,
                             int64_t Pp, const int32_t* __restrict__ pad_src) {
  const int e = blockIdx.y;
  const int64_t j = (int64_t)blockIdx.x * blockDim.x + threadIdx.x;
  if (j >= Pp) return;
  const float* th = theta + (int64_t)e * P;
  float v;
  if (j < P) v = th[j];
  else {
    const int32_t src = pad_src[j - P];
    v = src >= 0 ? th[src] : 0.f;
  }
  theta_pad[(int64_t)e * Pp + j] = v;
}
__global__ void k_fold_grad(float* __restrict__ grad_pad, int64_t Pp, const int32_t* __restrict__ fold_src,
                            float* __restrict__ grad, int64_t P) {
  const int e = blockIdx.y;
  const int64_t i = (int64_t)blockIdx.x * blockDim.x + threadIdx.x;
  if (i >= P) return;
  grad[(int64_t)e * P + i] = grad_pad[(int64_t)e * Pp + fold_src[i]];
}

struct AdamArgs {
  float* theta; float* m; float* v; float* grad;
  int64_t stride;
  int32_t P;
  int32_t off_shape;
  float lr, bc1, bc2;
  float prior_weight;
  float* loss; int64_t loss_stride; float loss_scale;
  int32_t apply;
  float* loss_raw;
  const StepState* st;
  int32_t keep_lo, keep_hi;
};

__global__ void k_step_advance(StepState* st) {
  if (threadIdx.x == 0 && blockIdx.x == 0) {
    const long long t = st->t + 1;
    st->t = t;
    st->col += 1;
    st->bc1 = (float)(1.0 - pow(0.9, (double)t));
    st->bc2 = (float)(1.0 - pow(0.999, (double)t));
  }
}

#ifndef BNF_ADAM_QUADS
#define BNF_ADAM_QUADS 4
#endif
__global__ __launch_bounds__(256) void k_adam_map(AdamArgs a) {
  __shared__ float red[4];
  const int e = blockIdx.y;
  const float bc1 = a.st ? a.st->bc1 : a.bc1, bc2 = a.st ? a.st->bc2 : a.bc2;
  float lp = 0.f;
#pragma unroll
  for (int qd = 0; qd < BNF_ADAM_QUADS; ++qd) {
  const int p0 = ((blockIdx.x * BNF_ADAM_QUADS + qd) * blockDim.x + threadIdx.x) * 4;
  if (p0 < a.P) {
    const int nv = min(4, a.P - p0);
    const int64_t i0 = (int64_t)e * a.stride + p0;
    float th[4], g[4], m[4], v[4];
    load4u(a.theta + i0, nv, th); load4u(a.grad + i0, nv, g);
    if (a.apply) { load4u(a.m + i0, nv, m); load4u(a.v + i0, nv, v); }
    const float ibc1 = 1.0f / bc1, ibc2 = 1.0f / bc2;
#pragma unroll
    for (int k = 0; k < 4; ++k) {
      if (a.prior_weight != 0.f && k < nv) {
        const float z = th[k] - ((p0 + k) == a.off_shape ? -1.5f : 0.f);
        const float az = fabsf(z);
        const float e = __builtin_amdgcn_exp2f(-1.44269504088896340736f * az);
        const float r = __builtin_amdgcn_rcpf(1.0f + e);
        g[k] += a.prior_weight * copysignf((1.0f - e) * r, z);
        lp += -az - 1.38629436111989061883f * __builtin_amdgcn_logf(1.0f + e);
      }
      if (a.apply) {
        m[k] = 0.9f * m[k] + 0.1f * g[k];
        v[k] = 0.999f * v[k] + 0.001f * g[k] * g[k];
        th[k] = th[k] - a.lr * (m[k] * ibc1) * __builtin_amdgcn_rcpf(__builtin_amdgcn_sqrtf(v[k] * ibc2) + 1e-8f);
        g[k] = 0.f;
      }
    }
    if (!(a.apply && p0 >= a.keep_lo && p0 < a.keep_hi)) store4u(a.grad + i0, nv, g);
    if (a.apply) {
      store4u(a.theta + i0, nv, th);
      store4u<true>(a.m + i0, nv, m);
      store4u<true>(a.v + i0, nv, v);
    }
  }
  }
  const float s = wave_sum(lp);
  if ((threadIdx.x & 63) == 0) red[threadIdx.x >> 6] = s;
  __syncthreads();
  if (threadIdx.x == 0 && a.prior_weight != 0.f) {
    const float t = -(a.prior_weight) * (red[0] + red[1] + red[2] + red[3]);
    atomicAdd(&a.loss[(int64_t)e * a.loss_stride + (a.st ? a.st->col : 0)], a.loss_scale * t);
    if (a.loss_raw) atomicAdd(&a.loss_raw[e], t);
  }
}

__device__ __forceinline__ float hw_exp_neg_abs(float x) { return __builtin_amdgcn_exp2f(-1.44269504088896340736f * fabsf(x)); }
__device__ __forceinline__ float hw_log1p_of_exp(float t) { return 0.69314718055994530942f * __builtin_amdgcn_logf(1.0f + t); }
__device__ __forceinline__ float hw_softplus(float x) { return fmaxf(x, 0.f) + hw_log1p_of_exp(hw_exp_neg_abs(x)); }
__device__ __forceinline__ float hw_sigmoid(float x) {
  const float t = hw_exp_neg_abs(x), r = __builtin_amdgcn_rcpf(1.0f + t);
  return x >= 0.f ? r : t * r;
}
__device__ __forceinline__ float vi_sigma(float rho) { return 1e-4f + hw_softplus(rho); }

struct ViSegs {
  int32_t n;
  int32_t lo[BNF_MAX_LAYERS + 2], hi[BNF_MAX_LAYERS + 2];
};
__global__ __launch_bounds__(256) void k_vi_sample(const float* __restrict__ mu,
                                                   const float* __restrict__ rho, int32_t P,
                                                   int32_t S, uint64_t seed, int64_t member_offset,
                                                   uint64_t step, uint32_t stream,
                                                   float* __restrict__ z, int64_t z_member_stride,
                                                   int64_t z_sample_stride, ViSegs segs,
                                                   const float* __restrict__ ext_eps = nullptr,
                                                   JaxNoise jn = JaxNoise{}) {
  const int e = blockIdx.y;
  const int lo = segs.lo[blockIdx.z], hi = segs.hi[blockIdx.z];
  const int u0 = ((lo + kEpsQuadPhase) & ~3) + (blockIdx.x * blockDim.x + threadIdx.x) * 4;
  const int p0 = u0 - kEpsQuadPhase;
  const int klo = max(0, lo - p0), khi = min(4, hi - p0);
  if (khi <= klo) return;
  const int64_t i = (int64_t)e * P + p0;
  float m[4], sg[4];
  load4w(mu + i, klo, khi, m);
  load4w(rho + i, klo, khi, sg);
#pragma unroll
  for (int k = 0; k < 4; ++k) sg[k] = vi_sigma(sg[k]);
  for (int s = 0; s < S; ++s) {
    Normal4 n;
    if (ext_eps) {
      load4w(ext_eps + ((int64_t)e * S + s) * P + p0, klo, khi, n.v);
    } else if (jn.keys) {
#pragma unroll
      for (int k = 0; k < 4; ++k) n.v[k] = (k >= klo && k < khi) ? jax_normal(jn, e, s, p0 + k) : 0.f;
    } else {
      n = vi_eps_quad(seed, (uint32_t)(member_offset + e), (uint32_t)s, (uint32_t)(u0 >> 2), step, stream);
    }
    float zv[4];
#pragma unroll
    for (int k = 0; k < 4; ++k) zv[k] = m[k] + sg[k] * n.v[k];
    store4w(z + (int64_t)e * z_member_stride + (int64_t)s * z_sample_stride + p0, klo, khi, zv);
  }
}

struct ViAdamArgs {
  float* mu; float* rho; float* m_mu; float* v_mu; float* m_rho; float* v_rho;
  float* grad;
  int32_t P, S, off_shape;
  uint64_t seed; int64_t member_offset; uint64_t step;
  float lr, bc1, bc2, kl_weight;
  float* loss; int64_t loss_stride;
  int32_t apply;
  float* gmu_out; float* grho_out;
  const float* ext_eps;
  JaxNoise jn;
  const float* z;
  int32_t n_keep;
  int32_t keep_lo[BNF_MAX_LAYERS], keep_hi[BNF_MAX_LAYERS];
// ... 465 lines not shown
```

bayesnf_amd/engine.py:

```python

from __future__ import annotations

import ctypes as C
import os

import numpy as np
import torch

from . import _native
from . import distributed
from .spec import NetSpec


_warned_default_dtype = False


def default_dtype(compute_dtype=None) -> str:
  global _warned_default_dtype
  if compute_dtype is None and 'BNF_DTYPE' not in os.environ and not _warned_default_dtype:
    _warned_default_dtype = True
    import warnings
    warnings.warn("bayesnf_amd: compute_dtype defaults to 'fp32_split' (f32 storage and epilogues, contractions as three "
                  "split-bf16 MFMAs: within SURVEY 8d's fp32 gates, 1.8x the exact chain). Pass compute_dtype='fp32' for the exact "
                  "f32 MFMA chain, 'bf16' (~3.5x faster again) or 'fp8' -- or set BNF_DTYPE.", stacklevel=3)
# ... 167 lines not shown
    means = means.contiguous().float()
    scales = scales.contiguous().float()
    q = np.asarray(list(quantiles), dtype=np.float32)
    out = torch.empty((len(q), means.shape[1]), dtype=torch.float32, device=self.device)
    qa = (C.c_float * len(q))(*q.tolist())
    _native.check(self.lib.bnf_normal_mixture_quantiles(
        self.handle, _ptr(means), _ptr(scales), means.shape[0], means.shape[1], qa,
        len(q), 1 if approximate else 0, _ptr(out)), 'bnf_normal_mixture_quantiles')
    return out

  def count_mixture_quantiles(self, loc: torch.Tensor, aux: torch.Tensor, quantiles):
    loc = loc.contiguous().float()
    aux = aux.contiguous().float()
    q = np.asarray(list(quantiles), dtype=np.float32)
    means = torch.empty_like(loc)
    out = torch.empty((len(q), loc.shape[1]), dtype=torch.float32, device=self.device)
    qa = (C.c_float * max(1, len(q)))(*q.tolist())
    _native.check(self.lib.bnf_count_mixture_quantiles(
        self.handle, _ptr(loc), _ptr(aux), loc.shape[0], loc.shape[1], qa, len(q),
        _ptr(means), _ptr(out)), 'bnf_count_mixture_quantiles')
    return means, out

  def debug_loss_and_grad(self, epoch=0, step=0):
    k = 2 if self.mode == 'vi' else 1
    grads = torch.empty((k * self.members, self.net.P), dtype=torch.float32, device=self.device)
    loss = torch.empty((self.members,), dtype=torch.float32, device=self.device)
    _native.check(self.lib.bnf_debug_loss_and_grad(self.handle, epoch, step, _ptr(grads),
                                                   _ptr(loss)), 'bnf_debug_loss_and_grad')
    torch.cuda.synchronize(self.device)
    g = grads.cpu().numpy()
    if self.mode == 'vi':
      g = g.reshape(2, self.members, self.net.P)
    return loss.cpu().numpy(), g

  def debug_row_index(self, epoch=0, step=0) -> np.ndarray:
    out = torch.empty((self.members, self.batch), dtype=torch.int32, device=self.device)
    _native.check(self.lib.bnf_debug_row_index(self.handle, epoch, step, _ptr(out)),
                  'bnf_debug_row_index')
    torch.cuda.synchronize(self.device)
    return out.cpu().numpy()

  def debug_vi_eps(self, step=0) -> np.ndarray:
    out = torch.empty((self.members, self.S, self.net.P), dtype=torch.float32, device=self.device)
    _native.check(self.lib.bnf_debug_vi_eps(self.handle, step, _ptr(out)), 'bnf_debug_vi_eps')
    torch.cuda.synchronize(self.device)
    return out.cpu().numpy()

  def set_vi_noise_keys(self, step_keys, draw_keys, leaf_offsets):
    if step_keys is None and draw_keys is None:
      self._vi_keys = None
      _native.check(self.lib.bnf_vi_noise_keys(self.handle, None, 0, None, 0, None, 0), 'bnf_vi_noise_keys')
      return
    up = lambda a: None if a is None else torch.from_numpy(np.ascontiguousarray(a, dtype=np.uint32).view(np.int32)).to(self.device)
    sk, dk = up(step_keys), up(draw_keys)
    lo = np.ascontiguousarray(leaf_offsets, dtype=np.int32)
    self._vi_keys = (sk, dk)
    _native.check(self.lib.bnf_vi_noise_keys(
        self.handle, None if sk is None else _ptr(sk), 0 if sk is None else int(step_keys.shape[0]),
        None if dk is None else _ptr(dk), 0 if dk is None else int(draw_keys.shape[0]),
        lo.ctypes.data_as(C.c_void_p), int(len(lo) - 1)), 'bnf_vi_noise_keys')

  def debug_vi_noise(self, eps):
    self._ext_eps = None if eps is None else eps.contiguous().float().to(self.device)
    _native.check(self.lib.bnf_debug_vi_noise(self.handle, None if eps is None else _ptr(self._ext_eps)),
                  'bnf_debug_vi_noise')

  def debug_poison_lds(self, pattern=0x7fc00000):
    _native.check(self.lib.bnf_debug_poison_lds(self.handle, int(pattern) & 0xffffffff), 'bnf_debug_poison_lds')

  def debug_activation(self, what: int) -> np.ndarray:
    ev = self.members * self.S
    if what == 0 or what == 400:
      shape = (ev, self.batch, self.net.F)
    elif what == 200:
      shape = (ev, self.batch)
    else:
      shape = (ev, self.batch, self.net.width)
    out = torch.empty(shape, dtype=torch.float32, device=self.device)
    _native.check(self.lib.bnf_debug_activation(self.handle, what, _ptr(out)),
                  'bnf_debug_activation')
    torch.cuda.synchronize(self.device)
    return out.cpu().numpy()

  def debug_gemm_nt(self, A: np.ndarray, Bt: np.ndarray) -> np.ndarray:
    A = torch.as_tensor(np.ascontiguousarray(A, dtype=np.float32)).to(self.device)
    Bt = torch.as_tensor(np.ascontiguousarray(Bt, dtype=np.float32)).to(self.device)
    Cout = torch.empty((A.shape[0], Bt.shape[0]), dtype=torch.float32, device=self.device)
    _native.check(self.lib.bnf_debug_gemm_nt(self.handle, _ptr(A), _ptr(Bt), A.shape[0],
                                             Bt.shape[0], A.shape[1], _ptr(Cout)),
                  'bnf_debug_gemm_nt')
    torch.cuda.synchronize(self.device)
    return Cout.cpu().numpy()

  def debug_gemm_tn(self, A: np.ndarray, B: np.ndarray) -> np.ndarray:
    A = torch.as_tensor(np.ascontiguousarray(A, dtype=np.float32)).to(self.device)
    B = torch.as_tensor(np.ascontiguousarray(B, dtype=np.float32)).to(self.device)
    Cout = torch.empty((A.shape[1], B.shape[1]), dtype=torch.float32, device=self.device)
    _native.check(self.lib.bnf_debug_gemm_tn(self.handle, _ptr(A), _ptr(B), A.shape[0], A.shape[1],
                                             B.shape[1], _ptr(Cout)), 'bnf_debug_gemm_tn')
    torch.cuda.synchronize(self.device)
    return Cout.cpu().numpy()

  def profile(self, kernel):
    arg = None if kernel is None else str(kernel).encode()
    _native.check(self.lib.bnf_profile_enable(self.handle, arg), 'bnf_profile_enable')

  def profile_read(self) -> dict:
    cap = 32
    n = C.c_int32(cap)
    names = (C.c_char_p * cap)()
    avg = (C.c_double * cap)()
    calls = (C.c_int64 * cap)()
    _native.check(self.lib.bnf_profile_read(self.handle, C.byref(n), names, avg, calls),
                  'bnf_profile_read')
    out = {}
    for i in range(n.value):
      name = names[i].decode()
      out[name] = dict(avg_ms=avg[i], calls=calls[i],
                       flops=self.lib.bnf_kernel_flops(self.handle, names[i]))
    return out
```

include/bnf.h:

```cpp
#ifndef BNF_H_
#define BNF_H_

#include <stddef.h>
#include <stdint.h>

#ifdef __cplusplus
extern "C" {
#endif

#define BNF_ABI_VERSION 6

#define BNF_MAX_INPUTS   8
#define BNF_MAX_GROUPS   12
#define BNF_MAX_LAYERS   8
#define BNF_MAX_FREQS    96
#define BNF_MAX_INTERACT 16

enum {
  BNF_OK = 0,
  BNF_ERR_INVALID = -1,
  BNF_ERR_NO_DEVICE = -2,
  BNF_ERR_HIP = -3,
  BNF_ERR_STATE = -4
};
// ... 22 lines not shown
  int32_t group_kind[BNF_MAX_GROUPS];
  int32_t group_arg[BNF_MAX_GROUPS];
  int32_t group_ncols[BNF_MAX_GROUPS];
  int32_t group_col0[BNF_MAX_GROUPS];
  int32_t group_scale_off[BNF_MAX_GROUPS];
  int32_t fourier_degree[BNF_MAX_INPUTS];
  float   input_scale[BNF_MAX_INPUTS];
  int32_t n_freqs;
  float   freq[BNF_MAX_FREQS];
  float   harmonic[BNF_MAX_FREQS];
  int32_t n_interact;
  int32_t interact[BNF_MAX_INTERACT][2];
  int32_t off_log_noise_scale, off_shape, off_inflated;
  int32_t off_bias[BNF_MAX_LAYERS + 1];
  int32_t off_kernel[BNF_MAX_LAYERS + 1];
  int32_t off_layer_scale[BNF_MAX_LAYERS];
  int32_t off_output_scale;
  int32_t off_lsa;
  int32_t off_act_weight;

  int64_t n_rows;
  int64_t batch;
  int32_t members;
  int64_t member_offset;
  int32_t vi_samples;
  int32_t forward_only;
  int32_t pipeline;
  float   learning_rate;
  float   prior_weight;
  float   kl_weight;
  uint64_t seed;
} bnf_config;

typedef struct bnf_handle bnf_handle;

int bnf_abi_version(void);
const char* bnf_last_error(void);

int bnf_create(const bnf_config* cfg, bnf_handle** out);
void bnf_destroy(bnf_handle* h);

size_t bnf_workspace_bytes(const bnf_handle* h);
size_t bnf_state_bytes(const bnf_handle* h);
size_t bnf_param_bytes(const bnf_handle* h);
size_t bnf_owned_bytes(const bnf_handle* h);

int bnf_bind(bnf_handle* h, void* params , void* opt_state ,
             void* workspace , const float* X ,
             const float* y , void* stream);

int bnf_init_params(bnf_handle* h, float log_noise_init);

int bnf_init_params_keys(bnf_handle* h, const uint32_t* leaf_keys, const int32_t* leaf_offsets, int32_t n_leaves,
                         float log_noise_init);

int bnf_train(bnf_handle* h, int64_t epoch0, int64_t num_epochs, float* losses );

int bnf_vi_posterior_draws(bnf_handle* h, int32_t n_draws, float* out );

int bnf_row_tables(bnf_handle* h, const int32_t* tables, int64_t epoch0, int64_t n_epochs);

int bnf_row_keys(bnf_handle* h, const uint32_t* keys, int64_t epoch0, int64_t n_epochs, int32_t rounds);

int bnf_vi_noise_keys(bnf_handle* h, const uint32_t* step_keys, int64_t n_steps, const uint32_t* draw_keys,
                      int64_t n_draws, const int32_t* leaf_offsets, int32_t n_leaves);

int bnf_forward(bnf_handle* h, const float* theta, int64_t n_members,
                const float* Xnew, int64_t n_rows, float* loc, float* aux);

int bnf_normal_mixture_quantiles(bnf_handle* h, const float* means, const float* scales,
                                 int64_t n_members, int64_t n_rows, const float* q,
                                 int32_t n_q, int32_t approximate, float* out);

int bnf_count_mixture_quantiles(bnf_handle* h, const float* loc, const float* aux,
                                int64_t n_members, int64_t n_rows, const float* q,
                                int32_t n_q, float* means, float* out);

int bnf_debug_loss_and_grad(bnf_handle* h, int64_t epoch, int64_t step,
                            float* grads, float* loss);
int bnf_debug_row_index(bnf_handle* h, int64_t epoch, int64_t step, int32_t* out);
int bnf_debug_vi_eps(bnf_handle* h, int64_t step, float* out);
int bnf_debug_vi_noise(bnf_handle* h, const float* eps);
int bnf_debug_activation(bnf_handle* h, int32_t what, float* out);
int bnf_debug_gemm_nt(bnf_handle* h, const float* A, const float* Bt, int32_t M,
                      int32_t N, int32_t K, float* C);

int bnf_debug_gemm_tn(bnf_handle* h, const float* A, const float* B, int32_t R, int32_t M,
                      int32_t N, float* C);

int bnf_debug_poison_lds(bnf_handle* h, uint32_t pattern);

int bnf_profile_enable(bnf_handle* h, const char* kernel);
int bnf_profile_read(bnf_handle* h, int32_t* n, const char** names, double* avg_ms,
                     int64_t* calls);
double bnf_kernel_flops(const bnf_handle* h, const char* name);

#define BNF_COMM_ID_BYTES 128
typedef struct bnf_comm bnf_comm;
int bnf_comm_available(void);
int bnf_comm_unique_id(void* id);
int bnf_comm_create(const void* id, int32_t world, int32_t rank, int32_t device, bnf_comm** out);
int bnf_allgather(bnf_comm* c, const void* send, void* recv, size_t bytes_per_rank, void* stream);
int bnf_comm_create_local(int32_t n, const int32_t* devices, bnf_comm** out);
int bnf_allgather_group(int32_t n, bnf_comm* const* comms, const void* const* send, void* const* recv,
                        size_t bytes_per_rank, void* const* streams);
void bnf_comm_destroy(bnf_comm* c);

#ifdef __cplusplus
}
#endif
#endif
```

Measured before the change: 35900 member-steps/s.

## Fuse Adam update and bf16 fragment repack into hidden-layer wgrad epilogue

After: 34510 member-steps/s. 0.961x the previous value.

```diff
diff --git a/bayesnf_amd/_native.py b/bayesnf_amd/_native.py
--- a/bayesnf_amd/_native.py
+++ b/bayesnf_amd/_native.py
@@ -24,7 +24,7 @@
     'bnf_workspace_bytes', 'bnf_state_bytes', 'bnf_param_bytes', 'bnf_owned_bytes', 'bnf_bind',
     'bnf_init_params', 'bnf_init_params_keys', 'bnf_train', 'bnf_row_tables', 'bnf_row_keys', 'bnf_vi_posterior_draws', 'bnf_vi_noise_keys', 'bnf_forward',
     'bnf_normal_mixture_quantiles', 'bnf_count_mixture_quantiles', 'bnf_debug_loss_and_grad',
-    'bnf_debug_row_index', 'bnf_debug_vi_eps', 'bnf_debug_vi_noise', 'bnf_debug_activation',
+    'bnf_debug_row_index', 'bnf_debug_vi_eps', 'bnf_debug_vi_noise', 'bnf_debug_activation', 'bnf_debug_weight_fragments',
     'bnf_debug_gemm_nt', 'bnf_debug_gemm_tn', 'bnf_debug_poison_lds', 'bnf_profile_enable', 'bnf_profile_read',
     'bnf_kernel_flops', 'bnf_comm_available', 'bnf_comm_unique_id', 'bnf_comm_create', 'bnf_allgather',
     'bnf_comm_create_local', 'bnf_allgather_group', 'bnf_comm_destroy')
@@ -119,6 +119,7 @@
   lib.bnf_init_params_keys.argtypes = [vp, vp, C.POINTER(C.c_int32), C.c_int32, C.c_float]
   lib.bnf_vi_noise_keys.argtypes = [vp, vp, i64, vp, i64, vp, C.c_int32]
   lib.bnf_debug_activation.argtypes = [vp, i32, vp]
+  lib.bnf_debug_weight_fragments.argtypes = [vp, i32, i32, vp]
   lib.bnf_debug_gemm_nt.argtypes = [vp, vp, vp, i32, i32, i32, vp]
   lib.bnf_debug_gemm_tn.argtypes = [vp, vp, vp, i32, i32, i32, vp]
   lib.bnf_profile_enable.argtypes = [vp, C.c_char_p]
diff --git a/bayesnf_amd/csrc/bnf_api.hip b/bayesnf_amd/csrc/bnf_api.hip
--- a/bayesnf_amd/csrc/bnf_api.hip
+++ b/bayesnf_amd/csrc/bnf_api.hip
@@ -53,6 +53,11 @@
 };
 
 static constexpr int64_t kAtPad = 128;
+
+struct FusedStep {
+  RingAdam fu;
+  float* loss; int64_t loss_stride; float loss_scale; float* loss_raw; const StepState* st;
+};
 
 struct bnf_handle {
   bnf_config cfg;
@@ -119,6 +124,9 @@
   float* dH0 = nullptr; float* out = nullptr; float* ybat = nullptr; float* loss_raw = nullptr;
   float* vacc = nullptr; float* dv = nullptr;
   bool vi_sample_pack = true, vi_keep_z = false;
+  bool fused_adam = true;
+  uint32_t frag_current = 0;
+  const FusedStep* fused = nullptr;
   bool panel = false;
   void* Wf[BNF_MAX_LAYERS]; void* Wb[BNF_MAX_LAYERS];
   void* park[BNF_MAX_LAYERS];
@@ -424,12 +432,32 @@
       EpiArgs ep2 = ep;
       ep2.ablate = h->ablate;
       LaunchScope ls(h, kid, st, true);
+      RingAdam fu{};
+      if constexpr (TAG == 1) {
+        if (h->fused && g.splitk == 1) {
+          static std::atomic<uint64_t> attr_done_a{0};
+          fu = h->fused->fu;
+          const int nm = g.n_multi > 1 ? g.n_multi : 1;
+          for (int k = 0; k < nm; ++k) {
+            const int32_t off = g.n_multi > 1 ? g.off_out_multi[k] : ep.off_out;
+            int l = 1;
+            while (l < h->L - 1 && h->nd.off_kernel[l] != off) ++l;
+            fu.wf[k] = h->Wf[l]; fu.wb[k] = h->Wb[l];
+            h->frag_current |= 1u << l;
+          }
+          ep2.loss = h->fused->loss; ep2.loss_stride = h->fused->loss_stride; ep2.loss_scale = h->fused->loss_scale;
+          ep2.loss_raw = h->fused->loss_raw; ep2.st = h->fused->st;
+          allow_lds(h, &gemm_tn_ring<TAG, true, 8, true>, kRgLds, &attr_done_a);
+          hipLaunchKernelGGL((gemm_tn_ring<TAG, true, 8, true>), dim3(blocks), dim3(512), kRgLds, st, g, ep2, fu);
+          return;
+        }
+      }
       if (g.splitk == 1) {
         allow_lds(h, &gemm_tn_ring<TAG, true>, kRgLds, &attr_done_s);
-        hipLaunchKernelGGL((gemm_tn_ring<TAG, true>), dim3(blocks), dim3(512), kRgLds, st, g, ep2);
+        hipLaunchKernelGGL((gemm_tn_ring<TAG, true>), dim3(blocks), dim3(512), kRgLds, st, g, ep2, fu);
       } else {
         allow_lds(h, &gemm_tn_ring<TAG, false>, kRgLds, &attr_done);
-        hipLaunchKernelGGL((gemm_tn_ring<TAG, false>), dim3(blocks), dim3(512), kRgLds, st, g, ep2);
+        hipLaunchKernelGGL((gemm_tn_ring<TAG, false>), dim3(blocks), dim3(512), kRgLds, st, g, ep2, fu);
       }
       return;
     }
@@ -794,11 +822,11 @@
   wgrad_join(h);
 }
 
-static PackJobs pack_jobs(const bnf_handle* h, int* n_tiles) {
+static PackJobs pack_jobs(const bnf_handle* h, int* n_tiles, bool hidden_current = false) {
   PackJobs jb{};
-  jb.n_layers = h->L; jb.W = h->W;
+  jb.n_layers = hidden_current ? 1 : h->L; jb.W = h->W;
   int tiles = 0;
-  for (int l = 0; l < h->L; ++l) {
+  for (int l = 0; l < jb.n_layers; ++l) {
     jb.off_kernel[l] = h->nd.off_kernel[l];
     jb.n_in[l] = (l == 0) ? h->F : h->W;
     jb.n_pad[l] = (l == 0) ? h->Fp : h->W;
@@ -806,7 +834,7 @@
     tiles += (jb.n_pad[l] / 64) * (h->W / 64);
     jb.wf[l] = h->Wf[l]; jb.wb[l] = h->Wb[l]; jb.batch[l] = h->pack_batch[l];
   }
-  jb.tile0[h->L] = tiles;
+  jb.tile0[jb.n_layers] = tiles;
   jb.fold0 = h->fold0 ? 1 : 0; jb.F0n = h->F; jb.off_bias0 = h->nd.off_bias[0]; jb.off_ls0 = h->nd.off_ls[0];
   for (int l = 0; l < h->L; ++l) { jb.wf8[l] = h->Wf8[l]; jb.wb8[l] = h->Wb8[l]; }
   jb.batch8 = (int64_t)h->W * h->W;
@@ -814,10 +842,10 @@
   return jb;
 }
 template <typename T>
-static void run_pack_fragments(bnf_handle* h, const float* theta, int nmem) {
+static void run_pack_fragments(bnf_handle* h, const float* theta, int nmem, bool hidden_current = false) {
   LaunchScope ls(h, KID_PACK);
   int tiles = 0;
-  const PackJobs jb = pack_jobs(h, &tiles);
+  const PackJobs jb = pack_jobs(h, &tiles, hidden_current);
   hipLaunchKernelGGL((k_pack_layers<T>), dim3((unsigned)tiles * (unsigned)nmem), dim3(256), 0, h->stream,
                      theta, (int64_t)h->Pf, jb, h->nd, h->scal);
 }
@@ -866,7 +894,10 @@
 static void run_panel(bnf_handle* h, const float* theta, int nmem, const RowSrc& rs, float c,
                       const LossSink& sink, bool fragments_packed = false) {
   const int64_t Bp = h->Bp;
-  if (!fragments_packed) run_pack_fragments<bf16_t>(h, theta, nmem);
+  if (!fragments_packed) {
+    const uint32_t hidden = ((1u << h->L) - 1u) & ~1u;
+    run_pack_fragments<bf16_t>(h, theta, nmem, h->L > 1 && (h->frag_current & hidden) == hidden);
+  }
   {
     LaunchScope ls(h, KID_FEAT);
     dim3 grid(cdiv(h->B, kFeatRows) * (unsigned)nmem);
@@ -1069,6 +1100,17 @@
   return BNF_OK;
 }
 
+static bool fused_step_ok(const bnf_handle* h, int nmem) {
+  if (!h->fused_adam || !h->panel || !h->bf16 || h->q8 || h->pad || h->overlap || h->ablate != 0 || h->adam_clear_all ||
+      h->L < 2 || h->cfg.mode != BNF_MODE_MAP)
+    return false;
+  for (int l = 1; l < h->L; ++l) {
+    const WgradPlan p = wgrad_plan(h, nmem, l);
+    if (p.kind != WG_RING || p.splitk != 1) return false;
+  }
+  return true;
+}
+
 template <typename T>
 static int step_map(bnf_handle* h, int64_t epoch, int64_t step, const LossSink& sink, bool apply) {
   if (const int prc = ensure_row_perm(h, epoch)) return prc;
@@ -1076,8 +1118,22 @@
   const int E = h->cfg.members;
   const float c = (float)((double)h->N / (double)h->B);
   const float* thf = fw_theta(h, h->params, E);
+  const int64_t t = h->adam_t + 1;
+  const float bc1 = (float)(1.0 - std::pow(0.9, (double)t)), bc2 = (float)(1.0 - std::pow(0.999, (double)t));
+  const bool fuse = apply && fused_step_ok(h, E);
+  FusedStep fs{};
+  if (fuse) {
+    fs.fu.theta = h->params; fs.fu.m = h->state; fs.fu.v = h->state + (int64_t)E * h->P; fs.fu.stride = h->P;
+    fs.fu.lr = h->cfg.learning_rate; fs.fu.bc1 = bc1; fs.fu.bc2 = bc2; fs.fu.prior_weight = h->cfg.prior_weight;
+    fs.fu.w_batch = (int64_t)h->W * h->W;
+    fs.loss = sink.loss; fs.loss_stride = sink.stride; fs.loss_scale = sink.scale; fs.loss_raw = sink.raw; fs.st = sink.st;
+  } else {
+    h->frag_current = 0;
+  }
   if (h->panel) {
+    h->fused = fuse ? &fs : nullptr;
     run_panel(h, thf, E, rs, c, sink);
+    h->fused = nullptr;
   } else {
     run_pack<T>(h, thf, E);
     run_forward<T>(h, thf, E, rs, h->X, h->stab, h->y, h->B, true);
@@ -1087,23 +1143,32 @@
   AdamArgs a{};
   a.theta = h->params; a.m = h->state; a.v = h->state + (int64_t)E * h->P; a.grad = h->grad;
   a.stride = h->P; a.P = h->P; a.off_shape = h->nd.off_shape;
-  const int64_t t = h->adam_t + 1;
   a.lr = h->cfg.learning_rate;
-  a.bc1 = (float)(1.0 - std::pow(0.9, (double)t));
-  a.bc2 = (float)(1.0 - std::pow(0.999, (double)t));
+  a.bc1 = bc1;
+  a.bc2 = bc2;
   a.prior_weight = h->cfg.prior_weight;
   a.loss = sink.loss; a.loss_stride = sink.stride; a.loss_scale = sink.scale;
   a.apply = apply ? 1 : 0; a.loss_raw = sink.raw; a.st = sink.st;
   a.keep_lo = a.keep_hi = 0;
-  if (!h->pad && !h->adam_clear_all && h->ablate == 0)
+  a.n_quads = (int32_t)cdiv(h->P, 4);
+  if (fuse) {
+    for (int l = 1; l < h->L; ++l) {
+      const int32_t lo = h->nd.off_kernel[l], hi = lo + h->W * h->W;
+      a.skip_lo[a.n_skip] = lo; a.skip_hi[a.n_skip] = hi;
+      a.skipq_lo[a.n_skip] = (lo + 3) / 4; a.skipq_hi[a.n_skip] = hi / 4;
+      a.n_quads -= a.skipq_hi[a.n_skip] - a.skipq_lo[a.n_skip];
+      ++a.n_skip;
+    }
+  } else if (!h->pad && !h->adam_clear_all && h->ablate == 0) {
     for (int l = 1; l < h->L; ++l)
       if (wgrad_splitk(h, E, l) == 1 && a.keep_hi == 0) {
         a.keep_lo = (h->nd.off_kernel[l] + 3) / 4 * 4;
         a.keep_hi = (h->nd.off_kernel[l] + h->W * h->W) / 4 * 4;
       }
+  }
   {
     LaunchScope ls(h, KID_ADAM);
-    hipLaunchKernelGGL(k_adam_map, dim3(cdiv(cdiv(h->P, 4), 256 * BNF_ADAM_QUADS), (unsigned)E), dim3(256), 0, h->stream, a);
+    hipLaunchKernelGGL(k_adam_map, dim3(cdiv(a.n_quads, 256 * BNF_ADAM_QUADS), (unsigned)E), dim3(256), 0, h->stream, a);
   }
   if (apply) h->adam_t = t;
   return BNF_OK;
@@ -1360,6 +1425,7 @@
   h->adam_clear_all = getenv("BNF_ADAM_CLEAR_ALL") != nullptr;
   if (const char* v = getenv("BNF_VI_SAMPLE_PACK")) h->vi_sample_pack = atoi(v) != 0;
   if (const char* v = getenv("BNF_VI_KEEP_Z")) h->vi_keep_z = atoi(v) != 0;
+  if (const char* v = getenv("BNF_FUSED_ADAM")) h->fused_adam = atoi(v) != 0;
   {
     int want = cfg->pipeline;
     if (const char* pf = getenv("BNF_PIPELINE")) want = atoi(pf);
@@ -1519,6 +1585,7 @@
   }
   h->bound = true;
   h->adam_t = 0;
+  h->frag_current = 0;
   h->vi_keys = h->vi_draw_keys = nullptr; h->vi_key_rows = h->vi_draw_rows = 0; h->vi_key_t0 = 0;
   h->row_tab = nullptr; h->row_tab_epochs = 0;
   h->row_keys = nullptr; h->row_keys_epochs = 0; h->perm_epoch = -1;
@@ -1541,6 +1608,7 @@
   HIPCHK(hipMemsetAsync(h->state, 0, bnf_state_bytes(h), h->stream));
   HIPCHK(hipGetLastError());
   h->adam_t = 0;
+  h->frag_current = 0;
   h->vi_keys = h->vi_draw_keys = nullptr; h->vi_key_rows = h->vi_draw_rows = 0; h->vi_key_t0 = 0;
   return BNF_OK;
 }
@@ -1568,6 +1636,7 @@
   HIPCHK(hipMemsetAsync(h->state, 0, bnf_state_bytes(h), h->stream));
   HIPCHK(hipGetLastError());
   h->adam_t = 0;
+  h->frag_current = 0;
   h->vi_keys = h->vi_draw_keys = nullptr; h->vi_key_rows = h->vi_draw_rows = 0; h->vi_key_t0 = 0;
   return BNF_OK;
 }
@@ -1581,6 +1650,7 @@
   const int E = h->cfg.members;
   HIPCHK(hipMemsetAsync(losses, 0, (size_t)E * num_epochs * 4, h->stream));
   int rc = BNF_OK;
+  h->frag_current = 0;
   if (h->cfg.mode == BNF_MODE_MAP) {
     const int64_t steps = h->N / h->B;
     const bool graph_ok = h->B >= h->N && !h->prof && !h->overlap && h->stream2 && num_epochs >= 8 &&
@@ -1592,6 +1662,8 @@
       st0.bc2 = (float)(1.0 - std::pow(0.999, (double)st0.t));
       HIPCHK(hipMemcpyAsync(h->step_state, &st0, sizeof(st0), hipMemcpyHostToDevice, h->stream));
       HIPCHK(hipStreamSynchronize(h->stream));
+      const bool fused_graph = h->bf16 && fused_step_ok(h, E);
+      if (fused_graph) run_pack_fragments<bf16_t>(h, h->params, E);
       if (!h->graph_exec || h->graph_cols != num_epochs || h->graph_losses != losses) {
         if (h->graph_exec) { (void)hipGraphExecDestroy(h->graph_exec); h->graph_exec = nullptr; }
         hipGraph_t graph = nullptr;
@@ -1603,6 +1675,7 @@
             return fail(BNF_ERR_HIP, "hipStreamBeginCapture: %s", hipGetErrorString(be));
         }
         LossSink sink{losses, num_epochs, 1.0f, nullptr, h->step_state};
+        if (fused_graph) h->frag_current = ((1u << h->L) - 1u) & ~1u;
         rc = h->bf16 ? step_map<bf16_t>(h, epoch0, 0, sink, true) : step_map<float>(h, epoch0, 0, sink, true);
         h->adam_t -= 1;
         hipLaunchKernelGGL(k_step_advance, dim3(1), dim3(1), 0, h->stream, h->step_state);
@@ -1617,6 +1690,7 @@
       }
       for (int64_t ep = 0; ep < num_epochs; ++ep) HIPCHK(hipGraphLaunch(h->graph_exec, h->stream));
       h->adam_t += num_epochs;
+      h->frag_current = 0;
       HIPCHK(hipGetLastError());
       return BNF_OK;
     }
@@ -1759,6 +1833,7 @@
   HIPCHK(hipSetDevice(h->cfg.device));
   const int E = h->cfg.members;
   int rc;
+  h->frag_current = 0;
   if (h->cfg.mode == BNF_MODE_MAP) {
     HIPCHK(hipMemsetAsync(h->loss_raw, 0, (size_t)h->Ev * 4, h->stream));
     HIPCHK(hipMemsetAsync(loss, 0, (size_t)E * 4, h->stream));
@@ -1904,6 +1979,16 @@
   return BNF_OK;
 }
 
+int bnf_debug_weight_fragments(bnf_handle* h, int32_t layer, int32_t backward, void* out) {
+  if (!h || !h->bound || !out) return fail(BNF_ERR_STATE, "not bound / null");
+  if (!h->panel || !h->bf16) return fail(BNF_ERR_STATE, "no fragment-major weights on this handle (row-panel pipeline only)");
+  if (layer < 0 || layer >= h->L) return fail(BNF_ERR_INVALID, "layer=%d", layer);
+  HIPCHK(hipSetDevice(h->cfg.device));
+  const void* src = backward ? h->Wb[layer] : h->Wf[layer];
+  HIPCHK(hipMemcpyAsync(out, src, (size_t)h->Ev * h->pack_batch[layer] * 2, hipMemcpyDeviceToDevice, h->stream));
+  return BNF_OK;
+}
+
 int bnf_debug_gemm_nt(bnf_handle* h, const float* A, const float* Bt, int32_t M, int32_t N, int32_t K,
                       float* C) {
   if (!h || !A || !Bt || !C) return fail(BNF_ERR_INVALID, "null");
diff --git a/bayesnf_amd/csrc/bnf_gemm.h b/bayesnf_amd/csrc/bnf_gemm.h
--- a/bayesnf_amd/csrc/bnf_gemm.h
+++ b/bayesnf_amd/csrc/bnf_gemm.h
@@ -3,6 +3,7 @@
 #include <type_traits>
 
 #include "bnf_device.h"
+#include "bnf_kernels.h"
 
 namespace bnf {
 
@@ -1253,8 +1254,15 @@
 
 constexpr int kRgRows = 32, kRgStages = 4, kRgOp = kRgRows * 512, kRgStage = 2 * kRgOp;
 constexpr int kRgLds = kRgStages * kRgStage;
-template <int TAG, bool SWAP, int NW = 8>
-__global__ __launch_bounds__(64 * NW, NW == 8 ? 2 : 1) void gemm_tn_ring(const GemmArgs g, const EpiArgs ep) {
+struct RingAdam {
+  float* theta; float* m; float* v;
+  int64_t stride;
+  float lr, bc1, bc2, prior_weight;
+  void* wf[BNF_MAX_LAYERS]; void* wb[BNF_MAX_LAYERS];
+  int64_t w_batch;
+};
+template <int TAG, bool SWAP, int NW = 8, bool ADAM = false>
+__global__ __launch_bounds__(64 * NW, NW == 8 ? 2 : 1) void gemm_tn_ring(const GemmArgs g, const EpiArgs ep, const RingAdam fu) {
   constexpr int TJ = NW == 8 ? 2 : 4;
   constexpr int QN = 16 / NW;
   extern __shared__ __attribute__((aligned(16))) char smem[];
@@ -1281,6 +1289,13 @@
 #pragma unroll
   for (int k = 0; k < 8; ++k)
     if (g.n_multi > 1 && which == k) { gA = g.A_multi[k]; gB = g.B_multi[k]; off_out = g.off_out_multi[k]; }
+  [[maybe_unused]] void* fwf = fu.wf[0];
+  [[maybe_unused]] void* fwb = fu.wb[0];
+  if constexpr (ADAM) {
+#pragma unroll
+    for (int k = 1; k < 8; ++k)
+      if (g.n_multi > 1 && which == k) { fwf = fu.wf[k]; fwb = fu.wb[k]; }
+  }
 
   const int nk_total = g.K / kRgRows;
   const int nk_per = (nk_total + g.splitk - 1) / g.splitk;
@@ -1442,6 +1457,106 @@
     }
   }
 
+  if constexpr (ADAM) {
+    static_assert(SWAP && NW == 8, "the ADAM epilogue is written for the swapped eight-wave form");
+    __syncthreads();
+    const float bc1 = ep.st ? ep.st->bc1 : fu.bc1, bc2 = ep.st ? ep.st->bc2 : fu.bc2;
+    const float ibc1 = 1.0f / bc1, ibc2 = 1.0f / bc2;
+    const int W = ep.ld_f32;
+    const int mw = m0 + wr * 128 + frow;
+    const int nw = n0 + wc * 64 + 4 * kg;
+    const int64_t pb = (int64_t)e * fu.stride + off_out + (int64_t)mw * W + nw;
+    float* th_p = fu.theta + pb;
+    float* m_p = fu.m + pb;
+    float* v_p = fu.v + pb;
+    char* tt = smem + wave * (128 * 64 * 2);
+    const int KS = W / 16;
+    bf16_t* wb_p = (bf16_t*)fwb + (int64_t)e * fu.w_batch;
+    bf16_t* wf_p = (bf16_t*)fwf + (int64_t)e * fu.w_batch;
+    float lp = 0.f;
+    struct Grp { f32x4 th[2], m[2], v[2]; };
+    auto gofs = [&](int gi) {
+      const int i = gi >> 2, j = (gi >> 1) & 1, t = gi & 1;
+      return (int64_t)(i * 32) * W + j * 32 + 16 * t;
+    };
+    auto gload = [&](Grp& x, int gi) {
+      const int64_t o = gofs(gi);
+#pragma unroll
+      for (int q = 0; q < 2; ++q) {
+        x.th[q] = *reinterpret_cast<const f32x4u*>(th_p + o + 8 * q);
+        x.m[q] = *reinterpret_cast<const f32x4u*>(m_p + o + 8 * q);
+        x.v[q] = *reinterpret_cast<const f32x4u*>(v_p + o + 8 * q);
+      }
+    };
+    auto gdo = [&](Grp& x, int gi, auto gi_tag) {
+      constexpr int GI = decltype(gi_tag)::value;
+      constexpr int i = GI >> 2, j = (GI >> 1) & 1, t = GI & 1;
+      const int64_t o = gofs(gi);
+      uint32_t pk[2][2];
+#pragma unroll
+      for (int q = 0; q < 2; ++q) {
+        constexpr int rg = 2 * t;
+        float th[4], gq[4], mm[4], vv[4];
+#pragma unroll
+        for (int k = 0; k < 4; ++k) {
+          th[k] = x.th[q][k]; mm[k] = x.m[q][k]; vv[k] = x.v[q][k];
+          gq[k] = acc[i][j][(rg + q) * 4 + k] * ep.scale;
+          adam_map_elem(th[k], gq[k], mm[k], vv[k], lp, 0.f, fu.prior_weight, true, fu.lr, ibc1, ibc2);
+        }
+        store4u(th_p + o + 8 * q, 4, th);
+        store4u<true>(m_p + o + 8 * q, 4, mm);
+        store4u<true>(v_p + o + 8 * q, 4, vv);
+        pk[q][0] = pack_bf16x2(th[0], th[1]);
+        pk[q][1] = pack_bf16x2(th[2], th[3]);
+        const int m_l = i * 32 + frow;
+#pragma unroll
+        for (int k = 0; k < 4; ++k) {
+          const int n_l = j * 32 + 16 * t + 8 * q + 4 * kg + k;
+          const uint32_t w16 = (k & 1) ? (pk[q][k >> 1] >> 16) : (pk[q][k >> 1] & 0xffffu);
+          *reinterpret_cast<uint16_t*>(tt + n_l * 256 + (((m_l >> 3) ^ (n_l & 15)) << 4) + (m_l & 7) * 2) = (uint16_t)w16;
+        }
+      }
+      uint32_t got[2];
+#pragma unroll
+      for (int d = 0; d < 2; ++d) got[d] = (uint32_t)__shfl_xor((int)(kg ? pk[0][d] : pk[1][d]), 32, 64);
+      const u32x4 frag = kg ? u32x4{got[0], got[1], pk[1][0], pk[1][1]} : u32x4{pk[0][0], pk[0][1], got[0], got[1]};
+      const int64_t f = (int64_t)((m0 + wr * 128 + i * 32) >> 5) * KS + ((n0 + wc * 64 + j * 32 + 16 * t) >> 4);
+      *reinterpret_cast<u32x4*>(wb_p + (f * 64 + lane) * 8) = frag;
+    };
+    Grp ga, gb;
+    gload(ga, 0);
+    auto pair = [&](auto gi_tag) {
+      constexpr int GI = decltype(gi_tag)::value;
+      gload(gb, GI + 1);
+      gdo(ga, GI, std::integral_constant<int, GI>{});
+      if constexpr (GI + 2 < 16) gload(ga, GI + 2);
+      gdo(gb, GI + 1, std::integral_constant<int, GI + 1>{});
+    };
+    pair(std::integral_constant<int, 0>{});  pair(std::integral_constant<int, 2>{});
+    pair(std::integral_constant<int, 4>{});  pair(std::integral_constant<int, 6>{});
+    pair(std::integral_constant<int, 8>{});  pair(std::integral_constant<int, 10>{});
+    pair(std::integral_constant<int, 12>{}); pair(std::integral_constant<int, 14>{});
+    asm volatile("" ::: "memory");
+    __builtin_amdgcn_wave_barrier();
+#pragma unroll
+    for (int nt = 0; nt < 2; ++nt)
+#pragma unroll
+      for (int ks = 0; ks < 8; ++ks) {
+        const int n_l = nt * 32 + frow;
+        const u32x4 frag = *reinterpret_cast<const u32x4*>(tt + n_l * 256 + (((ks * 2 + kg) ^ (n_l & 15)) << 4));
+        const int64_t f = (int64_t)(((n0 + wc * 64) >> 5) + nt) * KS + (((m0 + wr * 128) >> 4) + ks);
+        *reinterpret_cast<u32x4*>(wf_p + (f * 64 + lane) * 8) = frag;
+      }
+    if (fu.prior_weight != 0.f) {
+      const float s = wave_sum(lp);
+      if (lane == 0) {
+        const float t = -fu.prior_weight * s;
+        atomicAdd(&ep.loss[(int64_t)e * ep.loss_stride + (ep.st ? ep.st->col : 0)], ep.loss_scale * t);
+        if (ep.loss_raw) atomicAdd(&ep.loss_raw[e], t);
+      }
+    }
+    return;
+  }
   float* out = ep.out_f32 ? ep.out_f32 + (int64_t)e * ep.f32_batch
                           : ep.grad + (int64_t)e * ep.grad_stride + off_out;
   if constexpr (SWAP) {
diff --git a/bayesnf_amd/csrc/bnf_kernels.h b/bayesnf_amd/csrc/bnf_kernels.h
--- a/bayesnf_amd/csrc/bnf_kernels.h
+++ b/bayesnf_amd/csrc/bnf_kernels.h
@@ -599,7 +599,29 @@
   float* loss_raw;
   const StepState* st;
   int32_t keep_lo, keep_hi;
+  int32_t n_skip, n_quads;
+  int32_t skip_lo[BNF_MAX_LAYERS], skip_hi[BNF_MAX_LAYERS];
+  int32_t skipq_lo[BNF_MAX_LAYERS], skipq_hi[BNF_MAX_LAYERS];
 };
+
+__device__ __forceinline__ void adam_map_elem(float& th, float& g, float& m, float& v, float& lp, float loc,
+                                              float prior_weight, bool apply, float lr, float ibc1, float ibc2) {
+  asm volatile("" : "+v"(g));
+  if (prior_weight != 0.f) {
+    const float z = th - loc;
+    const float az = fabsf(z);
+    const float e = __builtin_amdgcn_exp2f(-1.44269504088896340736f * az);
+    const float r = __builtin_amdgcn_rcpf(1.0f + e);
+    g += prior_weight * copysignf((1.0f - e) * r, z);
+    lp += -az - 1.38629436111989061883f * __builtin_amdgcn_logf(1.0f + e);
+  }
+  if (apply) {
+    m = 0.9f * m + 0.1f * g;
+    v = 0.999f * v + 0.001f * g * g;
+    th = th - lr * (m * ibc1) * __builtin_amdgcn_rcpf(__builtin_amdgcn_sqrtf(v * ibc2) + 1e-8f);
+    g = 0.f;
+  }
+}
 
 __global__ void k_step_advance(StepState* st) {
   if (threadIdx.x == 0 && blockIdx.x == 0) {
@@ -621,30 +643,35 @@
   float lp = 0.f;
 #pragma unroll
   for (int qd = 0; qd < BNF_ADAM_QUADS; ++qd) {
-  const int p0 = ((blockIdx.x * BNF_ADAM_QUADS + qd) * blockDim.x + threadIdx.x) * 4;
-  if (p0 < a.P) {
+  int q = (blockIdx.x * BNF_ADAM_QUADS + qd) * blockDim.x + threadIdx.x;
+  const bool in_grid = q < a.n_quads;
+#pragma unroll
+  for (int r = 0; r < BNF_MAX_LAYERS; ++r)
+    if (r < a.n_skip && q >= a.skipq_lo[r]) q += a.skipq_hi[r] - a.skipq_lo[r];
+  const int p0 = q * 4;
+  if (in_grid && p0 < a.P) {
     const int nv = min(4, a.P - p0);
     const int64_t i0 = (int64_t)e * a.stride + p0;
+    bool edge = false;
+#pragma unroll
+    for (int r = 0; r < BNF_MAX_LAYERS; ++r)
+      if (r < a.n_skip) edge = edge || (p0 < a.skip_hi[r] && p0 + 4 > a.skip_lo[r]);
     float th[4], g[4], m[4], v[4];
     load4u(a.theta + i0, nv, th); load4u(a.grad + i0, nv, g);
     if (a.apply) { load4u(a.m + i0, nv, m); load4u(a.v + i0, nv, v); }
     const float ibc1 = 1.0f / bc1, ibc2 = 1.0f / bc2;
 #pragma unroll
     for (int k = 0; k < 4; ++k) {
-      if (a.prior_weight != 0.f && k < nv) {
-        const float z = th[k] - ((p0 + k) == a.off_shape ? -1.5f : 0.f);
-        const float az = fabsf(z);
-        const float e = __builtin_amdgcn_exp2f(-1.44269504088896340736f * az);
-        const float r = __builtin_amdgcn_rcpf(1.0f + e);
-        g[k] += a.prior_weight * copysignf((1.0f - e) * r, z);
-        lp += -az - 1.38629436111989061883f * __builtin_amdgcn_logf(1.0f + e);
+      bool mine = k < nv;
+      if (edge) {
+#pragma unroll
+        for (int r = 0; r < BNF_MAX_LAYERS; ++r)
+          if (r < a.n_skip) mine = mine && !(p0 + k >= a.skip_lo[r] && p0 + k < a.skip_hi[r]);
       }
-      if (a.apply) {
-        m[k] = 0.9f * m[k] + 0.1f * g[k];
-        v[k] = 0.999f * v[k] + 0.001f * g[k] * g[k];
-        th[k] = th[k] - a.lr * (m[k] * ibc1) * __builtin_amdgcn_rcpf(__builtin_amdgcn_sqrtf(v[k] * ibc2) + 1e-8f);
-        g[k] = 0.f;
-      }
+      if (mine)
+        adam_map_elem(th[k], g[k], m[k], v[k], lp, (p0 + k) == a.off_shape ? -1.5f : 0.f, a.prior_weight, a.apply != 0, a.lr,
+                      ibc1, ibc2);
+      else if (a.apply) g[k] = 0.f;
     }
     if (!(a.apply && p0 >= a.keep_lo && p0 < a.keep_hi)) store4u(a.grad + i0, nv, g);
     if (a.apply) {
diff --git a/bayesnf_amd/engine.py b/bayesnf_amd/engine.py
--- a/bayesnf_amd/engine.py
+++ b/bayesnf_amd/engine.py
@@ -273,6 +273,15 @@
     torch.cuda.synchronize(self.device)
     return out.cpu().numpy()
 
+  def debug_weight_fragments(self, layer: int, backward: bool) -> np.ndarray:
+    n_in = self.net.F if layer == 0 else self.net.width
+    n_pad = -(-n_in // 64) * 64
+    out = torch.empty((self.members * self.S, n_pad * self.net.width), dtype=torch.int16, device=self.device)
+    _native.check(self.lib.bnf_debug_weight_fragments(self.handle, int(layer), int(bool(backward)), _ptr(out)),
+                  'bnf_debug_weight_fragments')
+    torch.cuda.synchronize(self.device)
+    return out.cpu().numpy().view(np.uint16)
+
   def debug_gemm_nt(self, A: np.ndarray, Bt: np.ndarray) -> np.ndarray:
     A = torch.as_tensor(np.ascontiguousarray(A, dtype=np.float32)).to(self.device)
     Bt = torch.as_tensor(np.ascontiguousarray(Bt, dtype=np.float32)).to(self.device)
diff --git a/include/bnf.h b/include/bnf.h
--- a/include/bnf.h
+++ b/include/bnf.h
@@ -128,6 +128,8 @@
 int bnf_debug_vi_eps(bnf_handle* h, int64_t step, float* out);
 int bnf_debug_vi_noise(bnf_handle* h, const float* eps);
 int bnf_debug_activation(bnf_handle* h, int32_t what, float* out);
+int bnf_debug_weight_fragments(bnf_handle* h, int32_t layer, int32_t backward, void* out);
+
 int bnf_debug_gemm_nt(bnf_handle* h, const float* A, const float* Bt, int32_t M,
                       int32_t N, int32_t K, float* C);
 
```
